# palash1992/GEM

Hardware: NVIDIA H100
Metric: nodes/sec embedded at d=128 (higher is better)
Workload: dtype f32

## Files before the change

### gem_b200/csrc/apply_tc.cu

```cuda
#include "tc_common.cuh"

namespace gemb {

struct ApplyTcParams {
    int64_t n;
    const float *Q;
    const float *M;
    float *Out;
    int b1, b2, ldm, ldo;
    uint32_t a_lbo;
    uint32_t a_tile;
    uint32_t b_tile;
    uint32_t raw_slot;
};

template <int TILE_M, int NPAD>
__global__ void __launch_bounds__(384, 1) apply_tc_kernel(ApplyTcParams p) {
    extern __shared__ __align__(128) char smem[];
    __shared__ __align__(8) uint64_t s_full[2], s_tile_full, s_tile_free;
    const int tid = threadIdx.x, lane = tid & 31, warp = tid >> 5;
    const int kchunks = p.b1 / 4;
    const int ksteps = p.b1 / 8;
    const uint32_t a_sbo = 128u;
    const uint32_t b_lbo = 128u;
    const uint32_t b_sbo = (uint32_t)kchunks * 128u;
    char *raw_base = smem;
    char *a_hi = smem + 2 * (size_t)p.raw_slot, *a_lo = a_hi + p.a_tile;
    char *b_hi = a_lo + p.a_tile, *b_lo = b_hi + p.b_tile;

    if (tid == 0) {
        for (int i = 0; i < 2; i++) tc::mbar_init(tc::smem_u32(&s_full[i]), 1);
        tc::mbar_init(tc::smem_u32(&s_tile_full), 4);
        tc::mbar_init(tc::smem_u32(&s_tile_free), 8);
        asm volatile("fence.mbarrier_init.release.cluster;" ::: "memory");
    }
    for (int idx = tid; idx < NPAD * kchunks; idx += blockDim.x) {
        const int nn = idx % NPAD, kc = idx / NPAD;
        float4 v = make_float4(0.f, 0.f, 0.f, 0.f);
        if (nn < p.b2) {
            const float *m = p.M + (size_t)(4 * kc) * p.ldm + nn;
            v = make_float4(__ldg(m), __ldg(m + p.ldm), __ldg(m + 2 * (size_t)p.ldm), __ldg(m + 3 * (size_t)p.ldm));
        }
        uint4 hi, lo;
        tc::split_tf32(v, hi, lo);
        const uint32_t off = (uint32_t)(nn >> 3) * b_sbo + (uint32_t)(nn & 7) * 16u + (uint32_t)kc * b_lbo;
        *(uint4 *)(b_hi + off) = hi;
        *(uint4 *)(b_lo + off) = lo;
    }
    tc::fence_proxy_async();
    __syncthreads();

    const int64_t tiles_total = (p.n + TILE_M - 1) / TILE_M;
    const int nt = (int)((tiles_total - blockIdx.x + gridDim.x - 1) / gridDim.x);
    auto tile_row0 = [&](int t) { return ((int64_t)blockIdx.x + (int64_t)t * gridDim.x) * TILE_M; };
    auto tile_rows = [&](int t) { const int64_t r0 = tile_row0(t); return (int)(p.n - r0 < TILE_M ? p.n - r0 : TILE_M); };

    if (warp >= 8) {
        auto issue = [&](int t) {
            const int slot = t & 1;
            const uint32_t bytes = (uint32_t)tile_rows(t) * (uint32_t)p.b1 * 4u;
            const uint32_t bar = tc::smem_u32(&s_full[slot]);
            tc::mbar_expect_tx(bar, bytes);
            tc::bulk_g2s(tc::smem_u32(raw_base + (size_t)slot * p.raw_slot), p.Q + tile_row0(t) * p.b1, bytes, bar);
        };
        if (tid == 256) {
            if (nt > 0) issue(0);
            if (nt > 1) issue(1);
        }
        const int ltid = tid - 256;
        for (int t = 0; t < nt; t++) {
            const int slot = t & 1;
            const char *raw = raw_base + (size_t)slot * p.raw_slot;
            tc::mbar_wait(tc::smem_u32(&s_full[slot]), (uint32_t)(t >> 1) & 1);
            if (t >= 1) tc::mbar_wait(tc::smem_u32(&s_tile_free), (uint32_t)(t - 1) & 1);
            const int vr = tile_rows(t);
            for (int idx = ltid; idx < TILE_M * kchunks; idx += 128) {
                const int m = idx / kchunks, kc = idx - m * kchunks;
                float4 v = make_float4(0.f, 0.f, 0.f, 0.f);
                if (m < vr) v = *(const float4 *)(raw + ((size_t)m * p.b1 + 4 * kc) * 4);
                uint4 hi, lo;
                tc::split_tf32(v, hi, lo);
                const uint32_t off = (uint32_t)(m >> 3) * a_sbo + (uint32_t)(m & 7) * 16u + (uint32_t)kc * p.a_lbo;
                *(uint4 *)(a_hi + off) = hi;
                *(uint4 *)(a_lo + off) = lo;
            }
            tc::fence_proxy_async();
            __syncwarp();
            if (lane == 0) tc::mbar_arrive(tc::smem_u32(&s_tile_full));
            tc::named_sync(1, 128);
            if (tid == 256 && t + 2 < nt) issue(t + 2);
        }
    } else {
        const int wg = warp >> 2;
        const bool active = wg * 64 < TILE_M;
        float acc[NPAD / 2];
        const uint32_t a_off = (uint32_t)wg * 8u * a_sbo;
        for (int t = 0; t < nt; t++) {
            tc::mbar_wait(tc::smem_u32(&s_tile_full), (uint32_t)t & 1);
            __syncwarp();
            uint64_t dah = tc::make_desc(tc::smem_u32(a_hi) + a_off, p.a_lbo, a_sbo), dal = tc::make_desc(tc::smem_u32(a_lo) + a_off, p.a_lbo, a_sbo);
            uint64_t dbh = tc::make_desc(tc::smem_u32(b_hi), b_lbo, b_sbo), dbl = tc::make_desc(tc::smem_u32(b_lo), b_lbo, b_sbo);
            const uint64_t a_step = (uint64_t)((2u * p.a_lbo) >> 4), b_step = (uint64_t)((2u * b_lbo) >> 4);
            if (active) {
                tc::wgmma_fence();
                for (int ks = 0; ks < ksteps; ks++) {
                    tc::wgmma_tf32<NPAD>(acc, dah, dbh, ks > 0 ? 1u : 0u);
                    tc::wgmma_tf32<NPAD>(acc, dah, dbl, 1u);
                    tc::wgmma_tf32<NPAD>(acc, dal, dbh, 1u);
                    dah += a_step; dal += a_step; dbh += b_step; dbl += b_step;
                }
                tc::wgmma_commit();
                tc::wgmma_wait_all();
            }
            __syncwarp();
            if (lane == 0) tc::mbar_arrive(tc::smem_u32(&s_tile_free));
            if (!active) continue;
            const int vr = tile_rows(t);
            const int r0 = wg * 64 + (warp & 3) * 16 + (lane >> 2);
            float *orow = p.Out + tile_row0(t) * p.ldo;
#pragma unroll
            for (int j = 0; j < NPAD / 8; j++) {
                const int col = j * 8 + (lane & 3) * 2;
                if (col < p.b2) {
                    if (r0 < vr) *(float2 *)(orow + (size_t)r0 * p.ldo + col) = make_float2(acc[4 * j], acc[4 * j + 1]);
                    if (r0 + 8 < vr) *(float2 *)(orow + (size_t)(r0 + 8) * p.ldo + col) = make_float2(acc[4 * j + 2], acc[4 * j + 3]);
                }
            }
        }
    }
}

template <int TILE_M, int NPAD>
static int apply_tc_launch_t(gemb_ctx *ctx, const ApplyTcParams &p, int grid, size_t smem_bytes) {
    static size_t attr_bytes = 0;
    if (attr_bytes < smem_bytes) {
        GEMB_CUDA(cudaFuncSetAttribute(apply_tc_kernel<TILE_M, NPAD>, cudaFuncAttributeMaxDynamicSharedMemorySize, (int)smem_bytes));
        attr_bytes = smem_bytes;
    }
    apply_tc_kernel<TILE_M, NPAD><<<grid, 384, smem_bytes, ctx->stream>>>(p);
    GEMB_CUDA(cudaGetLastError());
    count_launch();
    return GEMB_OK;
}

template <int TILE_M>
static int apply_tc_dispatch(gemb_ctx *ctx, const ApplyTcParams &p, int npad, int grid, size_t smem_bytes) {
    switch (npad) {
        case 32: return apply_tc_launch_t<TILE_M, 32>(ctx, p, grid, smem_bytes);
        case 64: return apply_tc_launch_t<TILE_M, 64>(ctx, p, grid, smem_bytes);
        case 80: return apply_tc_launch_t<TILE_M, 80>(ctx, p, grid, smem_bytes);
        case 96: return apply_tc_launch_t<TILE_M, 96>(ctx, p, grid, smem_bytes);
        default: return apply_tc_launch_t<TILE_M, 128>(ctx, p, grid, smem_bytes);
    }
}

static int pad_width(int b) {
    const int widths[5] = {32, 64, 80, 96, 128};
    for (int w : widths) if (w >= b) return w;
    return 128;
}

static size_t apply_smem_bytes(int tile_m, int b1, int npad) {
    const size_t raw_slot = (size_t)tile_m * b1 * 4, a_tile = (size_t)(b1 / 4) * (16 * tile_m + 16);
    const size_t b_tile = (size_t)(npad / 8) * (b1 / 4) * 128;
    return 2 * raw_slot + 2 * a_tile + 2 * b_tile + 256;
}

int apply_tc_launch(gemb_ctx *ctx, int64_t n, const float *Q, int b1, const float *M, int ldm, int b2, float *Out, int ldo) {
    if (b1 % 8 || b2 % 4 || b1 > 128 || ldo < b2 || ldo % 4 || ((uintptr_t)Out & 15) || n <= 0) return GEMB_ERR_UNSUPPORTED;
    const int cfg[5][2] = {{128, 128}, {64, 128}, {128, 64}, {64, 64}, {64, 32}};
    int tile_m = 0, nbw = 0;
    for (const auto &c : cfg) {
        const int w = std::min(c[1], b2);
        if (apply_smem_bytes(c[0], b1, pad_width(w)) <= 226 * 1024) { tile_m = c[0]; nbw = w; break; }
    }
    if (!tile_m) return GEMB_ERR_UNSUPPORTED;
    const int64_t tiles = (n + tile_m - 1) / tile_m;
    int grid = ctx->sm_count;
    if (grid > tiles) grid = (int)tiles;
    for (int n0 = 0; n0 < b2; n0 += nbw) {
        ApplyTcParams p;
        const int w = std::min(nbw, b2 - n0), npad = pad_width(w);
        p.n = n; p.Q = Q; p.M = M + n0; p.Out = Out + n0; p.b1 = b1; p.b2 = w; p.ldm = ldm; p.ldo = ldo;
        p.a_lbo = 16u * (uint32_t)tile_m + 16u;
        p.a_tile = (uint32_t)(b1 / 4) * p.a_lbo;
        p.b_tile = (uint32_t)(npad / 8) * (uint32_t)(b1 / 4) * 128u;
        p.raw_slot = (uint32_t)((size_t)tile_m * b1 * 4);
        const size_t smem_bytes = apply_smem_bytes(tile_m, b1, npad);
        if (tile_m == 128) GEMB_TRY(apply_tc_dispatch<128>(ctx, p, npad, grid, smem_bytes));
        else GEMB_TRY(apply_tc_dispatch<64>(ctx, p, npad, grid, smem_bytes));
    }
    return GEMB_OK;
}

}
```

### gem_b200/csrc/gram_tc.cu

```cuda
#include "tc_common.cuh"

namespace gemb {

struct GramTcParams {
    int64_t n;
    const float *P, *Q;
    int ldp, ldq;
    int m0, n0, mb, nb;
    double *part;
    int ldg;
    int64_t part_stride;
    int stage_rows;
    uint32_t tile_bytes_a, tile_bytes_b;
    uint32_t raw_bytes_p, raw_bytes_q;
};

__device__ __forceinline__ void transform_unit(const char *raw, int ld, int c0, int w, int valid_rows, int k4, int j32,
                                               int lane, char *tile_hi, char *tile_lo, uint32_t lbo, uint32_t sbo) {
    const int mn = j32 * 32 + lane;
    if (mn >= w) return;
    const int k0 = k4 * 4;
    const float *src = (const float *)raw + (size_t)k0 * ld + c0 + mn;
    float4 v;
    v.x = (k0 + 0 < valid_rows) ? src[0] : 0.f;
    v.y = (k0 + 1 < valid_rows) ? src[(size_t)ld] : 0.f;
    v.z = (k0 + 2 < valid_rows) ? src[2 * (size_t)ld] : 0.f;
    v.w = (k0 + 3 < valid_rows) ? src[3 * (size_t)ld] : 0.f;
    uint4 hi, lo;
    tc::split_tf32(v, hi, lo);
    const uint32_t off = (uint32_t)(mn >> 3) * sbo + (uint32_t)(mn & 7) * 16u + (uint32_t)k4 * lbo;
    *(uint4 *)(tile_hi + off) = hi;
    *(uint4 *)(tile_lo + off) = lo;
}

template <bool QRAW, bool BSEP, int NPAD>
__global__ void __launch_bounds__(384, 1) gram_tc_kernel(GramTcParams p) {
    extern __shared__ __align__(128) char smem[];
    __shared__ __align__(8) uint64_t s_full[3], s_tile_full[2], s_tile_free[2];
    const int tid = threadIdx.x, lane = tid & 31, warp = tid >> 5;
    const int kblocks = p.stage_rows / 8;
    const int kquads = p.stage_rows / 4;
    const uint32_t lbo = 128u;
    const uint32_t sbo = (uint32_t)kquads * 128u;
    const uint32_t raw_stage = p.raw_bytes_p + (QRAW ? p.raw_bytes_q : 0);
    const uint32_t stage_bytes = 2 * p.tile_bytes_a + (BSEP ? 2 * p.tile_bytes_b : 0);
    char *raw_base = smem;
    char *tile_base = smem + 3 * (size_t)raw_stage;

    if (tid == 0) {
        for (int i = 0; i < 2; i++) { tc::mbar_init(tc::smem_u32(&s_tile_full[i]), 4); tc::mbar_init(tc::smem_u32(&s_tile_free[i]), 8); }
        for (int i = 0; i < 3; i++) tc::mbar_init(tc::smem_u32(&s_full[i]), 1);
        asm volatile("fence.mbarrier_init.release.cluster;" ::: "memory");
    }
    __syncthreads();

    const int64_t stages_total = (p.n + p.stage_rows - 1) / p.stage_rows;
    const int64_t per_cta = (stages_total + gridDim.x - 1) / gridDim.x;
    const int64_t s_begin = (int64_t)blockIdx.x * per_cta;
    const int64_t s_end = s_begin + per_cta < stages_total ? s_begin + per_cta : stages_total;
    const int nst = (int)(s_end > s_begin ? s_end - s_begin : 0);

    if (warp >= 8) {
        const int lw = warp - 8;
        auto issue = [&](int it) {
            const int slot = it % 3;
            const int64_t row0 = (s_begin + it) * p.stage_rows;
            const int64_t vr = p.n - row0 < p.stage_rows ? p.n - row0 : p.stage_rows;
            const uint32_t bytes_p = (uint32_t)(vr * p.ldp * 4), bytes_q = QRAW ? (uint32_t)(vr * p.ldq * 4) : 0u;
            const uint32_t bar = tc::smem_u32(&s_full[slot]);
            char *dst = raw_base + (size_t)slot * raw_stage;
            tc::mbar_expect_tx(bar, bytes_p + bytes_q);
            tc::bulk_g2s(tc::smem_u32(dst), p.P + row0 * p.ldp, bytes_p, bar);
            if (QRAW) tc::bulk_g2s(tc::smem_u32(dst + p.raw_bytes_p), p.Q + row0 * p.ldq, bytes_q, bar);
        };
        if (tid == 256)
            for (int it = 0; it < 3 && it < nst; it++) issue(it);
        for (int it = 0; it < nst; it++) {
            const int st = it & 1, slot = it % 3;
            char *base = tile_base + (size_t)st * stage_bytes;
            const char *raw = raw_base + (size_t)slot * raw_stage;
            tc::mbar_wait(tc::smem_u32(&s_full[slot]), (uint32_t)(it / 3) & 1);
            if (it >= 2) tc::mbar_wait(tc::smem_u32(&s_tile_free[st]), (uint32_t)((it >> 1) - 1) & 1);
            const int64_t row0 = (s_begin + it) * p.stage_rows;
            const int vr = (int)(p.n - row0 < p.stage_rows ? p.n - row0 : p.stage_rows);
            const int units_a = kquads * ((p.mb + 31) / 32);
#pragma unroll 3
            for (int u = lw; u < units_a; u += 4)
                transform_unit(raw, p.ldp, p.m0, p.mb, vr, u % kquads, u / kquads, lane, base, base + p.tile_bytes_a, lbo, sbo);
            if (BSEP) {
                const int units_b = kquads * ((p.nb + 31) / 32);
                char *qb = base + 2 * p.tile_bytes_a;
                const char *rb = QRAW ? raw + p.raw_bytes_p : raw;
                const int ldb = QRAW ? p.ldq : p.ldp;
#pragma unroll 3
                for (int u = lw; u < units_b; u += 4)
                    transform_unit(rb, ldb, p.n0, p.nb, vr, u % kquads, u / kquads, lane, qb, qb + p.tile_bytes_b, lbo, sbo);
            }
            tc::fence_proxy_async();
            __syncwarp();
            if (lane == 0) tc::mbar_arrive(tc::smem_u32(&s_tile_full[st]));
            tc::named_sync(1, 128);
            if (tid == 256 && it + 3 < nst) issue(it + 3);
        }
    } else {
        const int wg = warp >> 2;
        const bool active = wg * 64 < p.mb;
        float acc[NPAD / 2], racc[NPAD / 2];
#pragma unroll
        for (int i = 0; i < NPAD / 2; i++) racc[i] = 0.f;
        for (int it = 0; it < nst; it++) {
            const int st = it & 1;
            tc::mbar_wait(tc::smem_u32(&s_tile_full[st]), (uint32_t)(it >> 1) & 1);
            if (active) {
                const uint32_t a_hi = tc::smem_u32(tile_base + (size_t)st * stage_bytes), a_lo = a_hi + p.tile_bytes_a;
                const uint32_t b_hi = BSEP ? a_hi + 2 * p.tile_bytes_a : a_hi;
                const uint32_t b_lo = BSEP ? b_hi + p.tile_bytes_b : a_lo;
                const uint32_t a_off = (uint32_t)wg * 8u * sbo;
                uint64_t dah = tc::make_desc(a_hi + a_off, lbo, sbo), dal = tc::make_desc(a_lo + a_off, lbo, sbo);
                uint64_t dbh = tc::make_desc(b_hi, lbo, sbo), dbl = tc::make_desc(b_lo, lbo, sbo);
                const uint64_t step = (uint64_t)((2u * lbo) >> 4);
                tc::wgmma_fence();
                for (int kb = 0; kb < kblocks; kb++) {
                    tc::wgmma_tf32<NPAD>(acc, dah, dbh, kb > 0 ? 1u : 0u);
                    tc::wgmma_tf32<NPAD>(acc, dah, dbl, 1u);
                    tc::wgmma_tf32<NPAD>(acc, dal, dbh, 1u);
                    dah += step; dal += step; dbh += step; dbl += step;
                }
                tc::wgmma_commit();
                tc::wgmma_wait_all();
            }
            __syncwarp();
            if (lane == 0) tc::mbar_arrive(tc::smem_u32(&s_tile_free[st]));
            if (active) {
#pragma unroll
                for (int i = 0; i < NPAD / 2; i++) racc[i] += acc[i];
            }
        }
        if (active) {
            const int r0 = wg * 64 + (warp & 3) * 16 + (lane >> 2);
            double *dst = p.part + (size_t)blockIdx.x * p.part_stride + (size_t)p.m0 * p.ldg + p.n0;
#pragma unroll
            for (int i = 0; i < NPAD / 2; i++) {
                const int row = r0 + ((i >> 1) & 1) * 8, col = (i >> 2) * 8 + (lane & 3) * 2 + (i & 1);
                if (row < p.mb && col < p.nb) dst[(size_t)row * p.ldg + col] = (double)racc[i];
            }
        }
    }
}

template <bool QRAW, bool BSEP, int NPAD>
static int gram_tc_launch_t(gemb_ctx *ctx, const GramTcParams &p, int grid, size_t smem_bytes) {
    static size_t attr_bytes = 0;
    if (attr_bytes < smem_bytes) {
        GEMB_CUDA(cudaFuncSetAttribute(gram_tc_kernel<QRAW, BSEP, NPAD>, cudaFuncAttributeMaxDynamicSharedMemorySize, (int)smem_bytes));
        attr_bytes = smem_bytes;
    }
    gram_tc_kernel<QRAW, BSEP, NPAD><<<grid, 384, smem_bytes, ctx->stream>>>(p);
    GEMB_CUDA(cudaGetLastError());
    count_launch();
    return GEMB_OK;
}

template <bool QRAW, bool BSEP>
static int gram_tc_dispatch(gemb_ctx *ctx, const GramTcParams &p, int grid, size_t smem_bytes) {
    if (p.nb <= 32) return gram_tc_launch_t<QRAW, BSEP, 32>(ctx, p, grid, smem_bytes);
    if (p.nb <= 64) return gram_tc_launch_t<QRAW, BSEP, 64>(ctx, p, grid, smem_bytes);
    if (p.nb <= 80) return gram_tc_launch_t<QRAW, BSEP, 80>(ctx, p, grid, smem_bytes);
    if (p.nb <= 96) return gram_tc_launch_t<QRAW, BSEP, 96>(ctx, p, grid, smem_bytes);
    return gram_tc_launch_t<QRAW, BSEP, 128>(ctx, p, grid, smem_bytes);
}

int gram_tc_launch(gemb_ctx *ctx, int64_t n, const float *P, int b1, const float *Q, int b2, double *G) {
    const bool cross = (P != Q);
    if (b1 % 4 || b2 % 4 || n <= 0) return GEMB_ERR_UNSUPPORTED;
    const int bm = (b1 + 127) / 128, bn = (b2 + 127) / 128;
    const size_t cols_raw = (size_t)b1 + (cross ? b2 : 0);
    size_t cols_tile = 0;
    for (int i = 0; i < bm; i++)
        for (int j = 0; j < bn; j++) {
            const int mb = std::min(128, b1 - 128 * i), nb = std::min(128, b2 - 128 * j);
            const bool bsep = cross || i != j;
            cols_tile = std::max(cols_tile, (size_t)(mb + 7) / 8 * 8 + (bsep ? (size_t)(nb + 7) / 8 * 8 : 0));
        }
    const size_t bytes_per_row = 3 * 4 * cols_raw + 2 * 2 * 4 * cols_tile;
    int rows = (int)((176 * 1024) / bytes_per_row) / 8 * 8;
    if (rows > 64) rows = 64;
    if (rows < 8) return GEMB_ERR_UNSUPPORTED;
    const size_t sbo = (size_t)(rows / 4) * 128;
    const size_t raw_stage = (size_t)rows * cols_raw * 4;
    const size_t smem_bytes = 3 * raw_stage + 2 * cols_tile / 8 * 2 * sbo + 16 * sbo + 1024;
    if (smem_bytes > 226 * 1024) return GEMB_ERR_UNSUPPORTED;
    const int64_t stages_total = (n + rows - 1) / rows;
    int grid = ctx->sm_count;
    if (grid > stages_total) grid = (int)stages_total;
    double *part = nullptr;
    GEMB_TRY(red_scratch(ctx, (size_t)grid * b1 * b2, &part));
    GramTcParams p;
    p.n = n; p.P = P; p.Q = Q; p.ldp = b1; p.ldq = b2;
    p.part = part; p.ldg = b2; p.part_stride = (int64_t)b1 * b2;
    p.stage_rows = rows;
    p.raw_bytes_p = (uint32_t)(rows * b1 * 4);
    p.raw_bytes_q = (uint32_t)(rows * b2 * 4);
    for (int i = 0; i < bm; i++)
        for (int j = 0; j < bn; j++) {
            p.m0 = 128 * i; p.mb = std::min(128, b1 - p.m0);
            p.n0 = 128 * j; p.nb = std::min(128, b2 - p.n0);
            p.tile_bytes_a = (uint32_t)((p.mb + 7) / 8) * (uint32_t)(rows / 4) * 128u;
            p.tile_bytes_b = (uint32_t)((p.nb + 7) / 8) * (uint32_t)(rows / 4) * 128u;
            if (cross) GEMB_TRY((gram_tc_dispatch<true, true>(ctx, p, grid, smem_bytes)));
            else if (i != j) GEMB_TRY((gram_tc_dispatch<false, true>(ctx, p, grid, smem_bytes)));
            else GEMB_TRY((gram_tc_dispatch<false, false>(ctx, p, grid, smem_bytes)));
        }
    return sum_partials_launch(ctx, grid, (int64_t)b1 * b2, part, G);
}

}
```

### gem_b200/csrc/hope.cu

```cuda
#include "common.cuh"
#include <chrono>
#include "nccl_api.h"
#include <math.h>
#include <string.h>
#include <algorithm>
#include <numeric>

namespace gemb {

struct HopeWork {
    gemb_graph *g;
    gemb_ctx *c;
    int b;
    int64_t rows;
    int64_t shard;
    float *buf[5] = {nullptr, nullptr, nullptr, nullptr, nullptr};
    float *full = nullptr;
    double *G = nullptr, *G2 = nullptr, *w = nullptr, *Z = nullptr, *Zs = nullptr, *scal = nullptr;
    float *Minv = nullptr, *M1 = nullptr, *M2 = nullptr;
    int *rank_dev = nullptr;
    int64_t spmm_wide = 0, spmm_all = 0;
    bool halo = false;
    int64_t pushes = 0;
    double push_bytes_per_row = 0.0;
    bool wire_half = false;
    bool wire_full_now = false;
    bool blk_half[5] = {false, false, false, false, false};
    bool push_half() const { return wire_half && !wire_full_now; }
    int buf_index(const float *p) const { for (int i = 0; i < 5; i++) if (buf[i] == p) return i; return -1; }
    ~HopeWork() {
        if (!halo) for (auto p : buf) dfree(p);
        dfree(full); dfree(G); dfree(G2); dfree(w); dfree(Z); dfree(Zs); dfree(scal);
        dfree(Minv); dfree(M1); dfree(M2); dfree(rank_dev);
    }
};

struct HopeResult {
    int iters = 0, converged = 0, katz_terms = 0, algorithm = 0;
    double change = 0.0;
    float resid_max = -1.f, resid_est = -1.f;
    float *Xd = nullptr;
    float *Xalloc = nullptr;
    float *sig_dev = nullptr;
    double sigma_max = 0.0;
};

static int comm_allgather(HopeWork &W, const float *shard_src, int width) {
    NcclApi *api = nccl_api();
    if (!api) return GEMB_ERR_NCCL;
    GEMB_TRY(W.c->t_comm.begin(W.c->stream));
    ncclResult_t r = api->AllGather(shard_src, W.full, (size_t)W.shard * width, ncclFloat,
                                    (ncclComm_t)W.c->comm, W.c->stream);
    if (r != ncclSuccess) { set_error("ncclAllGather: %s", api->GetErrorString(r)); return GEMB_ERR_NCCL; }
    GEMB_TRY(W.c->t_comm.end(W.c->stream));
    return GEMB_OK;
}

static int comm_allreduce_f64(HopeWork &W, double *buf, size_t count) {
    if (W.c->nranks == 1) return GEMB_OK;
    NcclApi *api = nccl_api();
    if (!api) return GEMB_ERR_NCCL;
    GEMB_TRY(W.c->t_comm.begin(W.c->stream));
    ncclResult_t r = api->AllReduce(buf, buf, count, ncclDouble, ncclSum, (ncclComm_t)W.c->comm, W.c->stream);
    if (r != ncclSuccess) { set_error("ncclAllReduce: %s", api->GetErrorString(r)); return GEMB_ERR_NCCL; }
    GEMB_TRY(W.c->t_comm.end(W.c->stream));
    return GEMB_OK;
}

static int publish(HopeWork &W, const float *buf, int width) {
    if (!W.halo) return GEMB_OK;
    const int bi = W.buf_index(buf);
    GEMB_ARG(bi >= 0, "publish: not a work block");
    const bool half = W.push_half();
    GEMB_TRY(W.c->t_comm.begin(W.c->stream));
    GEMB_TRY(halo_push_launch(W.g, bi, width, half));
    GEMB_TRY(halo_barrier(W.g));
    GEMB_TRY(W.c->t_comm.end(W.c->stream));
    W.blk_half[bi] = half;
    W.pushes++;
    W.push_bytes_per_row += (half ? 2.0 : 4.0) * width;
    return GEMB_OK;
}

static int dist_spmm3(HopeWork &W, bool transpose, int width, float alpha, const float *Xshard, float gamma,
                      bool use_self, float delta, const float *X0, float *Y, bool timed, bool push_out = false) {
    if (W.halo) {
        gemb_csr_dev A = W.g->A;
        A.indices = W.g->halo.indices_ext;
        HaloPushArgs P;
        const int bo = W.buf_index(Y), bin = W.buf_index(Xshard);
        GEMB_ARG(bin >= 0, "spmm input is not a work block");
        const bool half_out = W.push_half();
        if (push_out) { GEMB_ARG(bo >= 0, "spmm output is not a work block"); halo_push_args(W.g, bo, &P, half_out); }
        if (timed) GEMB_TRY(W.c->t_spmm.begin(W.c->stream));
        GEMB_TRY(spmm3_launch(W.c, A, W.rows, width, alpha, Xshard, gamma, use_self ? Xshard : nullptr, delta, X0, Y,
                              push_out ? &P : nullptr, W.blk_half[bin] ? W.g->n_shard : 0));
        if (timed) { GEMB_TRY(W.c->t_spmm.end(W.c->stream)); W.spmm_wide++; }
        W.spmm_all++;
        if (push_out) {
            GEMB_TRY(W.c->t_comm.begin(W.c->stream));
            GEMB_TRY(halo_barrier(W.g));
            GEMB_TRY(W.c->t_comm.end(W.c->stream));
            W.blk_half[bo] = half_out;
            W.pushes++;
            W.push_bytes_per_row += (half_out ? 2.0 : 4.0) * width;
        }
        return GEMB_OK;
    }
    const float *Xfull = Xshard;
    if (W.c->nranks > 1) {
        GEMB_TRY(comm_allgather(W, Xshard, width));
        Xfull = W.full;
    }
    if (timed) GEMB_TRY(W.c->t_spmm.begin(W.c->stream));
    GEMB_TRY(spmm3_launch(W.c, transpose ? W.g->AT : W.g->A, W.rows, width, alpha, Xfull, gamma,
                          use_self ? Xshard : nullptr, delta, X0, Y));
    if (timed) { GEMB_TRY(W.c->t_spmm.end(W.c->stream)); W.spmm_wide++; }
    W.spmm_all++;
    return GEMB_OK;
}

static int dist_spmm(HopeWork &W, bool transpose, int width, float alpha, const float *Xshard,
                     const float *X0, float *Y, bool timed) {
    return dist_spmm3(W, transpose, width, alpha, Xshard, 0.f, false, 1.f, X0, Y, timed);
}

static int katz(HopeWork &W, bool transpose, float beta, int J, const float *in, float *out,
                float *t1, float *t2) {
    const float *cur = in;
    for (int m = 1; m <= J; m++) {
        if (m < J) {
            float *dst = (m & 1) ? t1 : t2;
            GEMB_TRY(dist_spmm3(W, transpose, W.b, beta, cur, 0.f, false, 1.f, in, dst, true, W.halo));
            cur = dst;
        } else {
            GEMB_TRY(dist_spmm(W, transpose, W.b, beta, cur, nullptr, out, true));
        }
    }
    return GEMB_OK;
}

static int gram_full(HopeWork &W, const float *P, const float *Q, double *G) {
    GEMB_TRY(W.c->t_dense.begin(W.c->stream));
    GEMB_TRY(gram_launch(W.c, W.rows, P, W.b, Q, W.b, G));
    GEMB_TRY(W.c->t_dense.end(W.c->stream));
    GEMB_TRY(comm_allreduce_f64(W, G, (size_t)W.b * W.b));
    return GEMB_OK;
}

static int cholqr_pass(HopeWork &W, double *G, const float *src, float *dst) {
    GEMB_TRY(W.c->t_dense.begin(W.c->stream));
    GEMB_TRY(chol_inverse_launch(W.c, W.b, G, W.Minv, W.rank_dev));
    GEMB_TRY(apply_launch(W.c, W.rows, src, W.b, W.Minv, W.b, W.b, dst, W.b));
    GEMB_TRY(W.c->t_dense.end(W.c->stream));
    return GEMB_OK;
}

static int cholqr2(HopeWork &W, const float *src, float *tmp, float *dst) {
    GEMB_TRY(gram_full(W, src, src, W.G));
    GEMB_TRY(cholqr_pass(W, W.G, src, tmp));
    GEMB_TRY(gram_full(W, tmp, tmp, W.G));
    GEMB_TRY(cholqr_pass(W, W.G, tmp, dst));
    return GEMB_OK;
}

__global__ void ritz_maps_kernel(int b, int k, const double *__restrict__ w, const double *__restrict__ Z,
                                 float *__restrict__ M1, float *__restrict__ M2, double p1, double p2,
                                 double rel_floor = 1e-28) {
    const int idx = blockIdx.x * blockDim.x + threadIdx.x;
    if (idx >= b * k) return;
    const int i = idx / k, j = idx - i * k;
    const double wmax = w[b - 1];
    const double th = w[b - k + j];
    const double z = Z[(size_t)i * b + (b - k + j)];
    double a = 0.0, c = 0.0;
    if (th > rel_floor * wmax && th > 0.0) { a = z * pow(th, p1); c = z * pow(th, p2); }
    M1[idx] = (float)a;
    M2[idx] = (float)c;
}

__global__ void sqrt_top_kernel(int b, int k, const double *__restrict__ w, float *__restrict__ sigma) {
    const int j = blockIdx.x * blockDim.x + threadIdx.x;
    if (j < k) { const double th = w[b - k + j]; sigma[j] = (float)(th > 0.0 ? sqrt(th) : 0.0); }
}

__global__ void coldiff_sumsq_kernel(int64_t n, int b, const float *__restrict__ A, const float *__restrict__ B,
                                     double *__restrict__ out) {
    const int j = threadIdx.x % b;
    const int rpb = blockDim.x / b;
    double acc = 0.0;
    for (int64_t r = (int64_t)blockIdx.x * rpb + threadIdx.x / b; r < n; r += (int64_t)gridDim.x * rpb) {
        const double d = (double)A[r * b + j] - (double)B[r * b + j];
        acc += d * d;
    }
    atomicAdd(out + j, acc);
}

__global__ void symmetrize_kernel(int b, double *__restrict__ T) {
    const int idx = blockIdx.x * blockDim.x + threadIdx.x;
    if (idx >= b * b) return;
    const int i = idx / b, j = idx - i * b;
    if (i < j) {
        const double v = 0.5 * (T[(size_t)i * b + j] + T[(size_t)j * b + i]);
        T[(size_t)i * b + j] = v;
        T[(size_t)j * b + i] = v;
    }
}

__global__ void axpby_kernel(int64_t count, float a, const float4 *__restrict__ P, float c,
                             const float4 *__restrict__ Q, float4 *__restrict__ Y) {
    for (int64_t i = (int64_t)blockIdx.x * blockDim.x + threadIdx.x; i < count; i += (int64_t)gridDim.x * blockDim.x) {
        const float4 p = P[i], q = Q[i];
        Y[i] = make_float4(a * p.x + c * q.x, a * p.y + c * q.y, a * p.z + c * q.z, a * p.w + c * q.w);
    }
}

__global__ void __launch_bounds__(256)
axpby_push_kernel(int64_t n_rows, int G, int rows_per_cta, float a, const float4 *__restrict__ P, float c,
                  const float4 *__restrict__ Q, float4 *__restrict__ Y, HaloPushArgs H) {
    const int lr = threadIdx.x / G, cc = threadIdx.x - lr * G;
    if (lr >= rows_per_cta) return;
    const int64_t row = (int64_t)blockIdx.x * rows_per_cta + lr;
    if (row >= n_rows) return;
    const float4 p = P[row * G + cc], q = Q[row * G + cc];
    const float4 v = make_float4(a * p.x + c * q.x, a * p.y + c * q.y, a * p.z + c * q.z, a * p.w + c * q.w);
    Y[row * G + cc] = v;
    halo_push_row(H, row, G, cc, v);
}

static int axpby_launch(HopeWork &W, float a, const float *P, float c, const float *Q, float *Y) {
    const int64_t count = W.rows * (int64_t)W.b / 4;
    if (W.halo) {
        const int G = W.b / 4, rpc = 256 / G, bo = W.buf_index(Y);
        GEMB_ARG(bo >= 0 && G <= 256, "axpby output is not a work block");
        HaloPushArgs H;
        const bool half = W.push_half();
        halo_push_args(W.g, bo, &H, half);
        W.blk_half[bo] = half;
        W.push_bytes_per_row += (half ? 2.0 : 4.0) * W.b;
        if (W.rows > 0) {
            axpby_push_kernel<<<(unsigned)((W.rows + rpc - 1) / rpc), 256, 0, W.c->stream>>>(
                W.rows, G, rpc, a, (const float4 *)P, c, (const float4 *)Q, (float4 *)Y, H);
            GEMB_CUDA(cudaGetLastError());
            count_launch();
        }
        GEMB_TRY(W.c->t_comm.begin(W.c->stream));
        GEMB_TRY(halo_barrier(W.g));
        GEMB_TRY(W.c->t_comm.end(W.c->stream));
        W.pushes++;
        return GEMB_OK;
    }
    if (count == 0) return GEMB_OK;
    int grid = W.c->sm_count * 8;
    if ((int64_t)grid * 256 > count) grid = (int)((count + 255) / 256);
    axpby_kernel<<<grid, 256, 0, W.c->stream>>>(count, a, (const float4 *)P, c, (const float4 *)Q, (float4 *)Y);
    GEMB_CUDA(cudaGetLastError());
    count_launch();
    return GEMB_OK;
}

__global__ void csr_rowsum_kernel(int64_t n, const int32_t *__restrict__ indptr, const float *__restrict__ vals,
                                  double *__restrict__ out) {
    double mx = 0.0, neg = 0.0;
    for (int64_t r = (int64_t)blockIdx.x * blockDim.x + threadIdx.x; r < n; r += (int64_t)gridDim.x * blockDim.x) {
        const int s = indptr[r], e = indptr[r + 1];
        double acc = 0.0;
        if (vals) {
            for (int i = s; i < e; i++) { const double v = vals[i]; acc += fabs(v); if (-v > neg) neg = -v; }
        } else acc = (double)(e - s);
        if (acc > mx) mx = acc;
    }
    for (int o = 16; o > 0; o >>= 1) {
        mx = fmax(mx, __shfl_xor_sync(0xffffffffu, mx, o));
        neg = fmax(neg, __shfl_xor_sync(0xffffffffu, neg, o));
    }
    if ((threadIdx.x & 31) == 0) {
        atomicMax((unsigned long long *)out, (unsigned long long)__double_as_longlong(mx));
        atomicMax((unsigned long long *)(out + 1), (unsigned long long)__double_as_longlong(neg));
    }
}

static int comm_allreduce_max_f64(HopeWork &W, double *buf, size_t count) {
    if (W.c->nranks == 1) return GEMB_OK;
    NcclApi *api = nccl_api();
    if (!api) return GEMB_ERR_NCCL;
    ncclResult_t r = api->AllReduce(buf, buf, count, ncclDouble, ncclMax, (ncclComm_t)W.c->comm, W.c->stream);
    if (r != ncclSuccess) { set_error("ncclAllReduce(max): %s", api->GetErrorString(r)); return GEMB_ERR_NCCL; }
    return GEMB_OK;
}

static int rowsum_bound(HopeWork &W, double *norm_inf, bool *nonneg) {
    gemb_ctx *c = W.c;
    GEMB_CUDA(cudaMemsetAsync(W.scal, 0, 2 * sizeof(double), c->stream));
    if (W.rows > 0) {
        csr_rowsum_kernel<<<c->sm_count * 8, 256, 0, c->stream>>>(W.rows, W.g->A.indptr, W.g->A.data, W.scal);
        GEMB_CUDA(cudaGetLastError());
        count_launch();
    }
    GEMB_TRY(comm_allreduce_max_f64(W, W.scal, 2));
    double h[2];
    GEMB_CUDA(cudaMemcpyAsync(h, W.scal, sizeof h, cudaMemcpyDeviceToHost, c->stream));
    GEMB_CUDA(cudaStreamSynchronize(c->stream));
    *norm_inf = h[0];
    *nonneg = (h[1] == 0.0);
    return GEMB_OK;
}

static int estimate_norm2(HopeWork &W, uint64_t seed, float *x, float *y, float *z, double *out) {
    gemb_ctx *c = W.c;
    gemb_graph *g = W.g;
    const int pw = 4;
    struct FullWire { HopeWork &w; bool old; FullWire(HopeWork &w_) : w(w_), old(w_.wire_full_now) { w.wire_full_now = true; } ~FullWire() { w.wire_full_now = old; } } fw(W);
    GEMB_TRY(randn_launch(c, W.rows, pw, seed ^ 0x5bd1e995u, (uint64_t)g->row0, x));
    double est = 0.0, prev = -1.0;
    for (int it = 0; it < 16; it++) {
        double h[2];
        GEMB_TRY(sumsq_launch(c, W.rows * pw, x, W.scal));
        GEMB_TRY(publish(W, x, pw));
        GEMB_TRY(dist_spmm3(W, false, pw, 1.f, x, 0.f, false, 1.f, nullptr, y, false, true));
        GEMB_TRY(dist_spmm(W, true, pw, 1.f, y, nullptr, z, false));
        GEMB_TRY(sumsq_launch(c, W.rows * pw, z, W.scal + 1));
        GEMB_TRY(comm_allreduce_f64(W, W.scal, 2));
        GEMB_CUDA(cudaMemcpyAsync(h, W.scal, sizeof h, cudaMemcpyDeviceToHost, c->stream));
        GEMB_CUDA(cudaStreamSynchronize(c->stream));
        if (!(h[0] > 0.0) || !(h[1] > 0.0)) { est = 0.0; break; }
        est = sqrt(sqrt(h[1] / h[0]));
        GEMB_TRY(scale_launch(c, W.rows * pw, (float)(1.0 / sqrt(h[1])), z));
        std::swap(x, z);
        if (prev > 0 && fabs(est - prev) <= 1e-3 * est && it >= 3) break;
        prev = est;
    }
    *out = est;
    return GEMB_OK;
}

static int probe_katz_terms(HopeWork &W, float beta, double katz_tol, uint64_t seed, float *x, float *y, int *J_out,
                            double *rho_est) {
    gemb_ctx *c = W.c;
    const int pw = 4, Jmax = 2048;
    int Jbest = 1;
    *rho_est = 0.0;
    for (int tr = 0; tr < 2; tr++) {
        GEMB_TRY(randn_launch(c, W.rows, pw, seed ^ (0x7f4a7c15u + tr), (uint64_t)W.g->row0, x));
        double peak = 0.0, prev = 0.0;
        int j = 0;
        bool done = false;
        for (j = 1; j <= Jmax; j++) {
            double h = 0.0;
            GEMB_TRY(dist_spmm(W, tr == 1, pw, beta, x, nullptr, y, false));
            GEMB_TRY(sumsq_launch(c, W.rows * pw, y, W.scal));
            GEMB_TRY(comm_allreduce_f64(W, W.scal, 1));
            GEMB_CUDA(cudaMemcpyAsync(&h, W.scal, sizeof h, cudaMemcpyDeviceToHost, c->stream));
            GEMB_CUDA(cudaStreamSynchronize(c->stream));
            const double nt = sqrt(h);
            if (prev > 0.0) *rho_est = std::max(*rho_est * (j > 8 ? 0.0 : 1.0), nt / prev / (double)beta);
            if (!(nt < 1e30)) break;
            peak = std::max(peak, nt);
            if (nt <= katz_tol * peak) { done = true; break; }
            prev = nt;
            std::swap(x, y);
        }
        if (!done) return GEMB_ERR_DIVERGE;
        Jbest = std::max(Jbest, j);
    }
    *J_out = std::min(4096, Jbest + Jbest / 8 + 2);
    return GEMB_OK;
}

struct Opts {
    int oversample = 16, max_iters = 30, min_iters = 2, katz_terms = 0, compute_residual = 0, verbose = 0;
    int algorithm = 0, cheb_degree = 8, stop_rule = 0, lanczos_basis = 0;
    int spectral_mode = 0;
    float tol = 1e-6f, katz_tol = 1e-7f, range_log2 = 8.f;
    uint64_t seed = 1234;
};

static int katz_terms_for(double beta, double nrm, double katz_tol) {
    const double x1 = beta * nrm * 1.02;
    if (x1 <= 1e-30) return 1;
    int J = (int)ceil(log(katz_tol) / log(x1));
    return std::max(1, std::min(J, 4096));
}

static int residual_check(HopeWork &W, float beta, int J, const float *P, const float *Qs, float *scr0, float *scr1,
                          float *scr2, const std::vector<int> &cols, double smax, float *out) {
    gemb_ctx *c = W.c;
    const int b = W.b;
    GEMB_TRY(katz(W, true, beta, J, P, scr0, scr1, scr2));
    GEMB_CUDA(cudaMemsetAsync(W.scal, 0, sizeof(double) * b, c->stream));
    const int threads = (256 / b) * b > 0 ? (256 / b) * b : b;
    coldiff_sumsq_kernel<<<c->sm_count * 4, threads, 0, c->stream>>>(W.rows, b, scr0, Qs, W.scal);
    GEMB_CUDA(cudaGetLastError());
    count_launch();
    GEMB_TRY(comm_allreduce_f64(W, W.scal, b));
    std::vector<double> rs(b);
    GEMB_CUDA(cudaMemcpyAsync(rs.data(), W.scal, sizeof(double) * b, cudaMemcpyDeviceToHost, c->stream));
    GEMB_CUDA(cudaStreamSynchronize(c->stream));
    double rm = 0.0;
    for (int j : cols) rm = std::max(rm, sqrt(rs[j]) / std::max(smax, 1e-300));
    *out = (float)rm;
    return GEMB_OK;
}

static int hope_general(HopeWork &W, const Opts &o, int d, float beta, int J, HopeResult &R) {
    gemb_ctx *c = W.c;
    const int b = W.b, k = d / 2;
    float *V = W.buf[0], *U = W.buf[1], *Wk = W.buf[2], *T1 = W.buf[3], *T2 = W.buf[4];
    R.algorithm = 1;
    R.katz_terms = J;
    GEMB_TRY(randn_launch(c, W.rows, b, o.seed, (uint64_t)W.g->row0, T1));
    GEMB_TRY(cholqr2(W, T1, T2, V));

    std::vector<double> theta(b), theta_prev(b, 0.0);
    for (int it = 1; it <= o.max_iters; it++) {
        R.iters = it;
        GEMB_TRY(katz(W, false, beta, J, V, U, T1, T2));
        GEMB_TRY(gram_full(W, U, U, W.G));
        GEMB_CUDA(cudaMemcpyAsync(W.G2, W.G, sizeof(double) * b * b, cudaMemcpyDeviceToDevice, c->stream));
        GEMB_TRY(c->t_dense.begin(c->stream));
        GEMB_TRY(eigh_launch(c, b, W.G2, W.w, W.Z, W.Zs, std::min(1e-5, std::max(1e-13, 1e-2 * (double)o.tol))));
        GEMB_TRY(c->t_dense.end(c->stream));
        GEMB_CUDA(cudaMemcpyAsync(theta.data(), W.w, sizeof(double) * b, cudaMemcpyDeviceToHost, c->stream));
        GEMB_CUDA(cudaStreamSynchronize(c->stream));
        const double tmax = std::max(theta[b - 1], 1e-300);
        double change = 0.0;
        for (int j = b - k; j < b; j++) {
            const double sj = sqrt(std::max(theta[j], 0.0)), sp = sqrt(std::max(theta_prev[j], 0.0));
            change = std::max(change, fabs(sj - sp) / std::max(sj, 1e-3 * sqrt(tmax)));
        }
        R.change = change;
        theta_prev = theta;
        if (o.verbose)
            fprintf(stderr, "[gemb_hope/general] it %d  sigma_max %.6g sigma_k %.6g  ritz change %.3g\n", it,
                    sqrt(tmax), sqrt(std::max(theta[b - k], 0.0)), change);
        if (it >= o.min_iters && change <= (double)o.tol) { R.converged = 1; break; }
        if (it == o.max_iters) break;
        GEMB_TRY(c->t_dense.begin(c->stream));
        ritz_maps_kernel<<<(b * b + 255) / 256, 256, 0, c->stream>>>(b, b, W.w, W.Z, W.M1, W.M2, -0.5, 0.5, 1e-10);
        GEMB_CUDA(cudaGetLastError());
        count_launch();
        GEMB_TRY(apply_launch(c, W.rows, U, b, W.M1, b, b, T1, b));
        GEMB_TRY(c->t_dense.end(c->stream));
        GEMB_TRY(katz(W, true, beta, J, T1, Wk, U, T2));
        GEMB_TRY(cholqr2(W, Wk, T1, V));
    }
    R.sigma_max = sqrt(std::max(theta[b - 1], 0.0));

    R.Xd = T1;
    if ((size_t)d > (size_t)b) {
        GEMB_CUDA(dmalloc(&R.Xalloc, sizeof(float) * (size_t)std::max<int64_t>(W.rows, 1) * d));
        R.Xd = R.Xalloc;
    }
    GEMB_TRY(c->t_dense.begin(c->stream));
    ritz_maps_kernel<<<(b * k + 255) / 256, 256, 0, c->stream>>>(b, k, W.w, W.Z, W.M1, W.M2, -0.25, 0.25);
    GEMB_CUDA(cudaGetLastError());
    count_launch();
    GEMB_TRY(apply_launch(c, W.rows, U, b, W.M1, k, k, R.Xd, d));
    GEMB_TRY(apply_launch(c, W.rows, V, b, W.M2, k, k, R.Xd + k, d));
    R.sig_dev = (float *)W.G2;
    sqrt_top_kernel<<<(k + 127) / 128, 128, 0, c->stream>>>(b, k, W.w, R.sig_dev);
    GEMB_CUDA(cudaGetLastError());
    count_launch();
    GEMB_TRY(c->t_dense.end(c->stream));

    if (o.compute_residual) {
        ritz_maps_kernel<<<(b * b + 255) / 256, 256, 0, c->stream>>>(b, b, W.w, W.Z, W.M1, W.M2, -0.5, 0.5);
        GEMB_CUDA(cudaGetLastError());
        count_launch();
        float *Pm = Wk, *Qs = nullptr, *Qalloc = nullptr, *STP = nullptr;
        const size_t blk = sizeof(float) * (size_t)W.shard * b;
        if (R.Xalloc) Qs = T1;
        else { GEMB_CUDA(dmalloc(&Qalloc, blk ? blk : 4)); GEMB_CUDA(cudaMemsetAsync(Qalloc, 0, blk, c->stream)); Qs = Qalloc; }
        GEMB_CUDA(dmalloc(&STP, blk ? blk : 4));
        GEMB_CUDA(cudaMemsetAsync(STP, 0, blk, c->stream));
        int s = apply_launch(c, W.rows, U, b, W.M1, b, b, Pm, b);
        if (s == GEMB_OK) s = apply_launch(c, W.rows, V, b, W.M2, b, b, Qs, b);
        std::vector<int> cols;
        for (int j = b - k; j < b; j++) cols.push_back(j);
        if (s == GEMB_OK) s = residual_check(W, beta, J, Pm, Qs, STP, U, T2, cols, R.sigma_max, &R.resid_max);
        dfree(STP);
        dfree(Qalloc);
        if (s != GEMB_OK) return s;
    }
    return GEMB_OK;
}

static int orth_rotated(HopeWork &W, const float *F, float *tmp, float *dst) {
    gemb_ctx *c = W.c;
    const int b = W.b;
    GEMB_TRY(gram_full(W, F, F, W.G));
    GEMB_TRY(c->t_dense.begin(c->stream));
    GEMB_TRY(small_gemm_launch(c, b, W.G, 0, W.Z, W.Zs, nullptr));
    GEMB_TRY(small_gemm_launch(c, b, W.Z, 1, W.Zs, W.G, nullptr));
    GEMB_TRY(chol_inverse_launch(c, b, W.G, W.Minv, W.rank_dev, W.G2));
    GEMB_TRY(small_gemm_launch(c, b, W.Z, 0, W.G2, nullptr, W.M1));
    GEMB_TRY(apply_launch(c, W.rows, F, b, W.M1, b, b, tmp, b));
    GEMB_TRY(c->t_dense.end(c->stream));
    GEMB_TRY(gram_full(W, tmp, tmp, W.G));
    GEMB_TRY(cholqr_pass(W, W.G, tmp, dst));
    return GEMB_OK;
}

__global__ void refill_cols_kernel(int64_t count, int b, const double *__restrict__ G, const float *__restrict__ Rn,
                                   float *__restrict__ V) {
    for (int64_t i = (int64_t)blockIdx.x * blockDim.x + threadIdx.x; i < count; i += (int64_t)gridDim.x * blockDim.x) {
        const int j = (int)(i % b);
        if (G[(size_t)j * b + j] < 0.5) V[i] = Rn[i];
    }
}

static int refill_dropped(HopeWork &W, float *V, float *s1, float *s2, uint64_t seed) {
    gemb_ctx *c = W.c;
    const int b = W.b;
    int rank = b;
    GEMB_CUDA(cudaMemcpyAsync(&rank, W.rank_dev, sizeof(int), cudaMemcpyDeviceToHost, c->stream));
    GEMB_CUDA(cudaStreamSynchronize(c->stream));
    if (rank >= b) return GEMB_OK;
    GEMB_TRY(randn_launch(c, W.rows, b, seed, (uint64_t)W.g->row0, s1));
    GEMB_TRY(gram_full(W, V, V, W.G));
    const int64_t count = W.rows * (int64_t)b;
    if (count > 0) {
        const int grid = (int)std::min<int64_t>((count + 255) / 256, (int64_t)c->sm_count * 8);
        refill_cols_kernel<<<grid, 256, 0, c->stream>>>(count, b, W.G, s1, V);
        GEMB_CUDA(cudaGetLastError());
        count_launch();
    }
    GEMB_TRY(gram_full(W, V, V, W.G));
    GEMB_TRY(cholqr_pass(W, W.G, V, s2));
    GEMB_TRY(gram_full(W, s2, s2, W.G));
    GEMB_TRY(cholqr_pass(W, W.G, s2, V));
    return GEMB_OK;
}

static inline double katz_f(double beta, double l) { return beta * l / (1.0 - beta * l); }
constexpr int GEMB_SWITCH_TO_LANCZOS = 1000;

static int hope_symmetric(HopeWork &W, const Opts &o, int d, float beta, double nrm, double hard_bound, HopeResult &R) {
    gemb_ctx *c = W.c;
    const int mode = o.spectral_mode;
    const int b = W.b, k = mode ? d : d / 2;
    R.algorithm = 2;
    R.katz_terms = 0;
    float *V = W.buf[0], *AV = W.buf[1];
    float *pool[3] = {W.buf[2], W.buf[3], W.buf[4]};
    const bool ritz_bound = nrm < 0.0;
    double bound = ritz_bound ? hard_bound * 1.02 + 1e-30 : nrm * 1.02 + 1e-30;

    bool careful = getenv("GEMB_WARMUP_CAREFUL") != nullptr;
    if (!careful) {
        W.wire_full_now = true;
        GEMB_TRY(randn_launch(c, W.rows, b, o.seed, (uint64_t)W.g->row0, pool[0]));
        GEMB_TRY(publish(W, pool[0], b));
        GEMB_TRY(dist_spmm3(W, false, b, 1.f, pool[0], 0.f, false, 1.f, nullptr, pool[1], true, W.halo));
        GEMB_TRY(dist_spmm3(W, false, b, 1.f, pool[1], 0.f, false, 1.f, nullptr, pool[2], true, W.halo));
        GEMB_TRY(dist_spmm(W, false, b, 1.f, pool[2], nullptr, AV, true));
        W.wire_full_now = false;
        GEMB_TRY(gram_full(W, AV, AV, W.G));
        GEMB_TRY(cholqr_pass(W, W.G, AV, pool[0]));
        int rank1 = b;
        GEMB_CUDA(cudaMemcpyAsync(&rank1, W.rank_dev, sizeof(int), cudaMemcpyDeviceToHost, c->stream));
        GEMB_CUDA(cudaStreamSynchronize(c->stream));
        if (rank1 < b) careful = true;
        else {
            GEMB_TRY(gram_full(W, pool[0], pool[0], W.G));
            GEMB_TRY(cholqr_pass(W, W.G, pool[0], V));
            GEMB_TRY(publish(W, V, b));
        }
    }
    if (careful) {
        GEMB_TRY(randn_launch(c, W.rows, b, o.seed, (uint64_t)W.g->row0, pool[0]));
        GEMB_TRY(cholqr2(W, pool[0], pool[1], V));
        GEMB_TRY(publish(W, V, b));
        for (int s = 0; s < 3; s++) {
            GEMB_TRY(dist_spmm(W, false, b, 1.f, V, nullptr, AV, true));
            GEMB_TRY(cholqr2(W, AV, pool[0], V));
            GEMB_TRY(publish(W, V, b));
        }
    }

    std::vector<double> lam(b), gval(b), th_sorted(b), th_prev(b, 0.0);
    std::vector<double> Wh(o.stop_rule == 1 ? (size_t)b * b : 0), Zr(o.stop_rule == 1 ? (size_t)b * b : 0);
    std::vector<int> order(b);
    struct Plan { bool valid = false; int deg = 0; double e = 0, c0 = 0, sigma1 = 0; } plan;

    auto run_filter = [&](const Plan &pl, float **out) -> int {
        double sigma = pl.sigma1;
        const double e = pl.e, c0 = pl.c0, tau2 = 2.0 / pl.sigma1;
        float *prev = V, *cur = pool[0];
        float *free_a = pool[1], *free_b = pool[2];
        GEMB_TRY(axpby_launch(W, (float)(sigma / e), AV, (float)(-sigma * c0 / e), V, cur));
        for (int i = 2; i <= pl.deg; i++) {
            const double sn = 1.0 / (tau2 - sigma);
            float *nxt = free_a;
            GEMB_TRY(dist_spmm3(W, false, b, (float)(2.0 * sn / e), cur, (float)(-2.0 * sn * c0 / e), true,
                                (float)(-sigma * sn), prev, nxt, true, i < pl.deg));
            sigma = sn;
            float *old_prev = prev;
            prev = cur;
            cur = nxt;
            if (old_prev == V) { free_a = free_b; free_b = nullptr; }
            else { free_a = old_prev; }
        }
        *out = cur;
        return GEMB_OK;
    };

    for (int it = 1; it <= o.max_iters; it++) {
        R.iters = it;
        GEMB_TRY(dist_spmm(W, false, b, 1.f, V, nullptr, AV, true));
        GEMB_TRY(gram_full(W, V, AV, W.G2));
        symmetrize_kernel<<<(b * b + 255) / 256, 256, 0, c->stream>>>(b, W.G2);
        GEMB_CUDA(cudaGetLastError());
        count_launch();
        GEMB_TRY(c->t_dense.begin(c->stream));
        GEMB_TRY(eigh_launch(c, b, W.G2, W.w, W.Z, W.Zs, std::min(1e-5, std::max(1e-13, 1e-2 * (double)o.tol))));
        GEMB_TRY(c->t_dense.end(c->stream));
        GEMB_CUDA(cudaMemcpyAsync(lam.data(), W.w, sizeof(double) * b, cudaMemcpyDeviceToHost, c->stream));
        GEMB_CUDA(cudaStreamSynchronize(c->stream));
        float *filtered = nullptr;
        if (ritz_bound) {
            double amax = 0.0;
            for (int i = 0; i < b; i++) amax = std::max(amax, fabs(lam[i]));
            bound = std::min(hard_bound * 1.02, 1.05 * amax) + 1e-30;
        }
        for (int i = 0; i < b; i++) {
            const double l = std::max(-bound, std::min(bound, lam[i]));
            gval[i] = mode ? (l + bound) : fabs(katz_f(beta, l));
        }
        std::iota(order.begin(), order.end(), 0);
        std::sort(order.begin(), order.end(), [&](int a, int c2) { return gval[a] > gval[c2]; });
        for (int i = 0; i < b; i++) th_sorted[i] = gval[order[i]] * gval[order[i]];
        const double tmax = std::max(th_sorted[0], 1e-300);
        double change = 0.0;
        for (int j = 0; j < k; j++) {
            const double sj = sqrt(th_sorted[j]), sp = sqrt(th_prev[j]);
            change = std::max(change, fabs(sj - sp) / std::max(sj, 1e-3 * sqrt(tmax)));
        }
        R.change = change;
        th_prev = th_sorted;
        if (it == 1 && !mode && o.algorithm == 0 && W.g->n >= 2048 && gval[order[k - 1]] < 0.33 * gval[order[0]] &&
            gval[order[std::min(b - 1, 3)]] < 0.7 * gval[order[0]])
            return GEMB_SWITCH_TO_LANCZOS;
        double stop_measure = change;
        if (o.stop_rule == 1) {
            GEMB_TRY(gram_full(W, AV, AV, W.G));
            GEMB_CUDA(cudaMemcpyAsync(Wh.data(), W.G, sizeof(double) * b * b, cudaMemcpyDeviceToHost, c->stream));
            GEMB_CUDA(cudaMemcpyAsync(Zr.data(), W.Z, sizeof(double) * b * b, cudaMemcpyDeviceToHost, c->stream));
            GEMB_CUDA(cudaStreamSynchronize(c->stream));
            double worst = 0.0;
            for (int j = 0; j < k; j++) {
                const int col = order[j];
                double q = 0.0;
                for (int r = 0; r < b; r++) {
                    double t = 0.0;
                    for (int s2 = 0; s2 < b; s2++) t += Wh[(size_t)r * b + s2] * Zr[(size_t)s2 * b + col];
                    q += Zr[(size_t)r * b + col] * t;
                }
                const double l = std::max(-bound, std::min(bound, lam[col]));
                const double r2 = std::max(q - lam[col] * lam[col], 0.0);
                const double fp = mode ? 1.0 : (double)beta / ((1.0 - beta * l) * (1.0 - beta * l));
                worst = std::max(worst, fp * sqrt(r2) / std::max(gval[order[0]], 1e-300));
            }
            stop_measure = worst;
            R.resid_est = (float)worst;
        }
        if (o.verbose)
            fprintf(stderr, "[gemb_hope/symmetric] it %d  sigma_max %.6g sigma_k %.6g  ritz change %.3g%s%.3g\n", it,
                    gval[order[0]], gval[order[k - 1]], change, o.stop_rule == 1 ? "  residual " : " ", o.stop_rule == 1 ? stop_measure : 0.0);
        if (it >= o.min_iters && stop_measure <= (double)o.tol) { R.converged = 1; break; }
        if (it == o.max_iters) break;

        const double tau = gval[order[b - 1]];
        double hi = mode ? std::max(-bound, std::min(bound, lam[order[b - 1]])) : tau / ((double)beta * (1.0 + tau));
        double lo = mode ? -bound : (tau < 1.0 ? -tau / ((double)beta * (1.0 - tau)) : -bound);
        lo = std::max(lo, -bound);
        hi = std::min(hi, bound);
        if (hi - lo < 2e-3 * bound) { const double mid = 0.5 * (hi + lo); lo = mid - 1e-3 * bound; hi = mid + 1e-3 * bound; }
        Plan np;
        np.valid = true;
        np.e = 0.5 * (hi - lo);
        np.c0 = 0.5 * (hi + lo);
        const double aL = (mode || lam[order[0]] >= np.c0) ? bound : -bound;
        np.sigma1 = np.e / (aL - np.c0);
        const double xL = fabs(aL - np.c0) / np.e;
        const double growth = xL + sqrt(std::max(xL * xL - 1.0, 0.0));
        np.deg = o.cheb_degree;
        const double range_log2 = getenv("GEMB_CHEB_RANGE_LOG2") ? atof(getenv("GEMB_CHEB_RANGE_LOG2")) : (double)o.range_log2;
        if (growth > 1.0 + 1e-9) np.deg = std::min(np.deg, (int)floor(log(2.0 * exp2(range_log2)) / log(growth)));

        if (!filtered) {
            if (np.deg < 2) {
                GEMB_TRY(orth_rotated(W, AV, pool[0], V));
                GEMB_TRY(refill_dropped(W, V, pool[0], pool[1], o.seed + 7919ull * (uint64_t)it));
                GEMB_TRY(publish(W, V, b));
                plan = np;
                continue;
            }
            GEMB_TRY(run_filter(np, &filtered));
        }
        plan = np;
        float *tmp = nullptr;
        for (float *cand : {pool[0], pool[1], pool[2], AV})
            if (cand != filtered) { tmp = cand; break; }
        GEMB_TRY(orth_rotated(W, filtered, tmp, V));
        GEMB_TRY(refill_dropped(W, V, tmp, filtered, o.seed + 7919ull * (uint64_t)it));
        GEMB_TRY(publish(W, V, b));
    }

    if (mode) {
        std::vector<double> Zh((size_t)b * b);
        GEMB_CUDA(cudaMemcpyAsync(Zh.data(), W.Z, sizeof(double) * b * b, cudaMemcpyDeviceToHost, c->stream));
        GEMB_CUDA(cudaStreamSynchronize(c->stream));
        std::vector<float> M1((size_t)b * k), ev(k);
        for (int j = 0; j < k; j++) {
            const int col = order[j];
            ev[j] = (float)std::max(-bound, std::min(bound, lam[col]));
            for (int i = 0; i < b; i++) M1[(size_t)i * k + j] = (float)Zh[(size_t)i * b + col];
        }
        R.sigma_max = gval[order[0]];
        GEMB_CUDA(cudaMemcpyAsync(W.M1, M1.data(), sizeof(float) * b * k, cudaMemcpyHostToDevice, c->stream));
        R.sig_dev = (float *)W.G2;
        GEMB_CUDA(cudaMemcpyAsync(R.sig_dev, ev.data(), sizeof(float) * k, cudaMemcpyHostToDevice, c->stream));
        GEMB_CUDA(cudaStreamSynchronize(c->stream));
        R.Xd = pool[0];
        GEMB_TRY(c->t_dense.begin(c->stream));
        GEMB_TRY(apply_launch(c, W.rows, V, b, W.M1, k, k, R.Xd, k));
        GEMB_TRY(c->t_dense.end(c->stream));
        return GEMB_OK;
    }
    std::vector<int> sel(order.begin(), order.begin() + k);
    std::reverse(sel.begin(), sel.end());
    std::vector<double> Zh((size_t)b * b);
    GEMB_CUDA(cudaMemcpyAsync(Zh.data(), W.Z, sizeof(double) * b * b, cudaMemcpyDeviceToHost, c->stream));
    GEMB_CUDA(cudaStreamSynchronize(c->stream));
    std::vector<float> M1((size_t)b * k), M2((size_t)b * k), sig(k);
    for (int j = 0; j < k; j++) {
        const int col = sel[j];
        const double l = std::max(-bound, std::min(bound, lam[col]));
        const double f = katz_f(beta, l), sg = fabs(f), rt = sqrt(sg);
        sig[j] = (float)sg;
        for (int i = 0; i < b; i++) {
            const double z = Zh[(size_t)i * b + col];
            M2[(size_t)i * k + j] = (float)(z * rt);
            M1[(size_t)i * k + j] = (float)((f < 0 ? -z : z) * rt);
        }
    }
    R.sigma_max = gval[order[0]];
    GEMB_CUDA(cudaMemcpyAsync(W.M1, M1.data(), sizeof(float) * b * k, cudaMemcpyHostToDevice, c->stream));
    GEMB_CUDA(cudaMemcpyAsync(W.M2, M2.data(), sizeof(float) * b * k, cudaMemcpyHostToDevice, c->stream));
    R.sig_dev = (float *)W.G2;
    GEMB_CUDA(cudaMemcpyAsync(R.sig_dev, sig.data(), sizeof(float) * k, cudaMemcpyHostToDevice, c->stream));
    GEMB_CUDA(cudaStreamSynchronize(c->stream));
    R.Xd = pool[0];
    if ((size_t)d > (size_t)b) {
        GEMB_CUDA(dmalloc(&R.Xalloc, sizeof(float) * (size_t)std::max<int64_t>(W.rows, 1) * d));
        R.Xd = R.Xalloc;
    }
    GEMB_TRY(c->t_dense.begin(c->stream));
    GEMB_TRY(apply_launch(c, W.rows, V, b, W.M1, k, k, R.Xd, d));
    GEMB_TRY(apply_launch(c, W.rows, V, b, W.M2, k, k, R.Xd + k, d));
    GEMB_TRY(c->t_dense.end(c->stream));

    if (o.compute_residual) {
        const int J = katz_terms_for(beta, ritz_bound ? bound / 1.02 : nrm, o.katz_tol);
        std::vector<float> MP((size_t)b * b, 0.f), MQ((size_t)b * b, 0.f);
        for (int col = 0; col < b; col++) {
            const double l = std::max(-bound, std::min(bound, lam[col]));
            const double f = katz_f(beta, l);
            for (int i = 0; i < b; i++) {
                const double z = Zh[(size_t)i * b + col];
                MP[(size_t)i * b + col] = (float)(f < 0 ? -z : z);
                MQ[(size_t)i * b + col] = (float)(z * fabs(f));
            }
        }
        float *dMP = nullptr, *dMQ = nullptr, *Palloc = nullptr, *Q = nullptr, *STP = nullptr;
        const size_t blk = sizeof(float) * (size_t)W.shard * b;
        GEMB_CUDA(dmalloc(&dMP, sizeof(float) * b * b));
        GEMB_CUDA(dmalloc(&dMQ, sizeof(float) * b * b));
        float *P = AV;
        if (!W.halo) { GEMB_CUDA(dmalloc(&Palloc, blk ? blk : 4)); GEMB_CUDA(cudaMemsetAsync(Palloc, 0, blk, c->stream)); P = Palloc; }
        GEMB_CUDA(dmalloc(&Q, blk ? blk : 4));
        GEMB_CUDA(dmalloc(&STP, blk ? blk : 4));
        GEMB_CUDA(cudaMemsetAsync(Q, 0, blk, c->stream));
        GEMB_CUDA(cudaMemsetAsync(STP, 0, blk, c->stream));
        GEMB_CUDA(cudaMemcpyAsync(dMP, MP.data(), sizeof(float) * b * b, cudaMemcpyHostToDevice, c->stream));
        GEMB_CUDA(cudaMemcpyAsync(dMQ, MQ.data(), sizeof(float) * b * b, cudaMemcpyHostToDevice, c->stream));
        W.wire_full_now = true;
        int s = apply_launch(c, W.rows, V, b, dMP, b, b, P, b);
        if (s == GEMB_OK) s = apply_launch(c, W.rows, V, b, dMQ, b, b, Q, b);
        if (s == GEMB_OK) s = publish(W, P, b);
        if (s == GEMB_OK) s = residual_check(W, beta, J, P, Q, STP, W.halo ? pool[1] : AV, W.halo ? pool[2] : pool[1], sel, R.sigma_max, &R.resid_max);
        cudaStreamSynchronize(c->stream);
        dfree(dMP); dfree(dMQ); dfree(Palloc); dfree(Q); dfree(STP);
        if (s != GEMB_OK) return s;
    }
    return GEMB_OK;
}

__global__ void put_cols_kernel(int64_t n, int w, const float *__restrict__ src, float *__restrict__ dst, int ldd, int col0) {
    for (int64_t i = (int64_t)blockIdx.x * blockDim.x + threadIdx.x; i < n * w; i += (int64_t)gridDim.x * blockDim.x) {
        const int64_t r = i / w;
        const int cc = (int)(i - r * w);
        dst[r * ldd + col0 + cc] = src[i];
    }
}
__global__ void reverse_put_kernel(int64_t n, int w, const float *__restrict__ src, int lds, float *__restrict__ dst, int ldd, int col_last) {
    for (int64_t i = (int64_t)blockIdx.x * blockDim.x + threadIdx.x; i < n * w; i += (int64_t)gridDim.x * blockDim.x) {
        const int64_t r = i / w;
        const int q = (int)(i - r * w);
        dst[r * ldd + col_last - q] = src[r * lds + q];
    }
}
__global__ void f64_to_f32_kernel(int count, const double *__restrict__ a, float *__restrict__ o) {
    const int i = blockIdx.x * blockDim.x + threadIdx.x;
    if (i < count) o[i] = (float)a[i];
}
__global__ void axpy_kernel(int64_t count, float a, const float *__restrict__ X, float *__restrict__ Y, int accumulate) {
    for (int64_t i = (int64_t)blockIdx.x * blockDim.x + threadIdx.x; i < count; i += (int64_t)gridDim.x * blockDim.x)
        Y[i] = accumulate ? fmaf(a, X[i], Y[i]) : a * X[i];
}

static int hope_lanczos(HopeWork &W, const Opts &o, int d, float beta, double hard_bound, HopeResult &R) {
    gemb_ctx *c = W.c;
    const int k = d / 2, p = 16, cw = 64;
    const int64_t rows = W.rows, shard = W.shard;
    R.algorithm = 3;
    R.katz_terms = 0;
    const int k_keep = (k + p + p - 1) / p * p;
    int m_max = o.lanczos_basis > 0 ? o.lanczos_basis : std::max(2 * k_keep, 160);
    m_max = (m_max + p - 1) / p * p;
    GEMB_ARG(m_max >= k_keep + 2 * p && m_max <= 1024, "algorithm3_basis");
    const int nchunk = (m_max + cw - 1) / cw;
    const int mt = m_max + p;
    const size_t chunk_bytes = sizeof(float) * (size_t)shard * cw;
    std::vector<float *> Q(nchunk, nullptr), Qn((k_keep + cw - 1) / cw, nullptr);
    struct Free { std::vector<float *> *a, *b; float *t[3]; double *g[3]; float *m32;
                  ~Free() { for (auto x : *a) dfree(x); for (auto x : *b) dfree(x); for (auto x : t) dfree(x); for (auto x : g) dfree(x); dfree(m32); } }
        guard{&Q, &Qn, {nullptr, nullptr, nullptr}, {nullptr, nullptr, nullptr}, nullptr};
    for (auto &q : Q) { GEMB_CUDA(dmalloc(&q, chunk_bytes ? chunk_bytes : 4)); GEMB_CUDA(cudaMemsetAsync(q, 0, chunk_bytes, c->stream)); }
    for (auto &q : Qn) { GEMB_CUDA(dmalloc(&q, chunk_bytes ? chunk_bytes : 4)); }
    float *Vcur = W.buf[0], *Wb = W.buf[1], *Tb = W.buf[2], *Tmp64 = nullptr;
    GEMB_CUDA(dmalloc(&guard.t[0], chunk_bytes ? chunk_bytes : 4));
    Tmp64 = guard.t[0];
    double *Gd = nullptr, *Td = nullptr, *Yd = nullptr;
    GEMB_CUDA(dmalloc(&guard.g[0], sizeof(double) * (size_t)cw * cw)); Gd = guard.g[0];
    GEMB_CUDA(dmalloc(&guard.g[1], sizeof(double) * (size_t)mt * mt)); Td = guard.g[1];
    GEMB_CUDA(dmalloc(&guard.g[2], sizeof(double) * (size_t)mt * mt)); Yd = guard.g[2];
    GEMB_CUDA(dmalloc(&guard.m32, sizeof(float) * (size_t)cw * cw));
    float *M32 = guard.m32;
    double *wd = nullptr, *Zs = nullptr;
    GEMB_CUDA(dmalloc(&wd, sizeof(double) * mt));
    GEMB_CUDA(dmalloc(&Zs, sizeof(double) * (size_t)mt * mt));
    struct Free2 { double *a, *b; ~Free2() { dfree(a); dfree(b); } } guard2{wd, Zs};

    const int grid_el = c->sm_count * 8;
    auto gram_ar = [&](const float *P, int b1, const float *Qp, int b2, double *G) -> int {
        GEMB_TRY(c->t_dense.begin(c->stream));
        GEMB_TRY(gram_launch(c, rows, P, b1, Qp, b2, G));
        GEMB_TRY(c->t_dense.end(c->stream));
        return comm_allreduce_f64(W, G, (size_t)b1 * b2);
    };
    std::vector<double> Rh((size_t)p * p), R1((size_t)p * p), R2((size_t)p * p), Ginv((size_t)p * p);
    auto cholqr_p = [&](float *src, float *scratch, double *Rout) -> int {
        for (int pass = 0; pass < 2; pass++) {
            GEMB_TRY(gram_ar(src, p, src, p, W.G));
            GEMB_TRY(c->t_dense.begin(c->stream));
            GEMB_TRY(chol_inverse_launch(c, p, W.G, W.Minv, W.rank_dev, W.G2));
            GEMB_TRY(apply_launch(c, rows, src, p, W.Minv, p, p, scratch, p));
            GEMB_TRY(c->t_dense.end(c->stream));
            GEMB_CUDA(cudaMemcpyAsync(src, scratch, sizeof(float) * (size_t)rows * p, cudaMemcpyDeviceToDevice, c->stream));
            GEMB_CUDA(cudaMemcpyAsync(Ginv.data(), W.G2, sizeof(double) * p * p, cudaMemcpyDeviceToHost, c->stream));
            GEMB_CUDA(cudaStreamSynchronize(c->stream));
            std::vector<double> &Rt = pass == 0 ? R1 : R2;
            std::fill(Rt.begin(), Rt.end(), 0.0);
            for (int j = 0; j < p; j++) {
                if (Ginv[(size_t)j * p + j] == 0.0) continue;
                Rt[(size_t)j * p + j] = 1.0 / Ginv[(size_t)j * p + j];
                for (int i = j - 1; i >= 0; i--) {
                    if (Ginv[(size_t)i * p + i] == 0.0) continue;
                    double sacc = 0.0;
                    for (int l = i + 1; l <= j; l++) sacc += Ginv[(size_t)i * p + l] * Rt[(size_t)l * p + j];
                    Rt[(size_t)i * p + j] = -sacc / Ginv[(size_t)i * p + i];
                }
            }
        }
        for (int i = 0; i < p; i++)
            for (int j = 0; j < p; j++) {
                double a = 0.0;
                for (int l = 0; l < p; l++) a += R2[(size_t)i * p + l] * R1[(size_t)l * p + j];
                Rout[(size_t)i * p + j] = a;
            }
        return GEMB_OK;
    };

    std::vector<double> T((size_t)mt * mt, 0.0), Hcol((size_t)m_max * p), Hc((size_t)cw * p), theta(m_max), Y((size_t)m_max * m_max);
    std::vector<double> fabsv(m_max);
    std::vector<int> order(m_max);
    GEMB_TRY(randn_launch(c, rows, p, o.seed, (uint64_t)W.g->row0, Vcur));
    GEMB_TRY(cholqr_p(Vcur, Tb, Rh.data()));
    int m = 0, restarts = 0, steps = 0;
    double bound = hard_bound * 1.02 + 1e-30;
    const int max_steps = std::max(o.max_iters, 1) * (m_max / p);
    bool done = false;
    while (!done) {
        put_cols_kernel<<<grid_el, 256, 0, c->stream>>>(rows, p, Vcur, Q[m / cw], cw, m % cw);
        GEMB_CUDA(cudaGetLastError());
        count_launch();
        const int j0 = m;
        m += p;
        steps++;
        GEMB_TRY(publish(W, Vcur, p));
        GEMB_TRY(dist_spmm3(W, false, p, 1.f, Vcur, 0.f, false, 1.f, nullptr, Wb, true, false));
        std::fill(Hcol.begin(), Hcol.end(), 0.0);
        const int nc_live = (m + cw - 1) / cw;
        for (int pass = 0; pass < 2; pass++) {
            for (int cc = 0; cc < nc_live; cc++) {
                GEMB_TRY(gram_ar(Q[cc], cw, Wb, p, Gd));
                GEMB_TRY(c->t_dense.begin(c->stream));
                f64_to_f32_kernel<<<(cw * p + 255) / 256, 256, 0, c->stream>>>(cw * p, Gd, M32);
                GEMB_CUDA(cudaGetLastError());
                GEMB_TRY(apply_launch(c, rows, Q[cc], cw, M32, p, p, Tb, p));
                axpy_kernel<<<grid_el, 256, 0, c->stream>>>(rows * (int64_t)p, -1.f, Tb, Wb, 1);
                GEMB_CUDA(cudaGetLastError());
                count_launch(2);
                GEMB_TRY(c->t_dense.end(c->stream));
                GEMB_CUDA(cudaMemcpyAsync(Hc.data(), Gd, sizeof(double) * cw * p, cudaMemcpyDeviceToHost, c->stream));
                GEMB_CUDA(cudaStreamSynchronize(c->stream));
                for (int r = 0; r < cw && cc * cw + r < m; r++)
                    for (int q = 0; q < p; q++) Hcol[(size_t)(cc * cw + r) * p + q] += Hc[(size_t)r * p + q];
            }
        }
        for (int r = 0; r < m; r++)
            for (int q = 0; q < p; q++) {
                const double v = Hcol[(size_t)r * p + q];
                T[(size_t)r * mt + j0 + q] = v;
                T[(size_t)(j0 + q) * mt + r] = v;
            }
        for (int a2 = 0; a2 < p; a2++)
            for (int b2 = a2 + 1; b2 < p; b2++) {
                const double v = 0.5 * (T[(size_t)(j0 + a2) * mt + j0 + b2] + T[(size_t)(j0 + b2) * mt + j0 + a2]);
                T[(size_t)(j0 + a2) * mt + j0 + b2] = v;
                T[(size_t)(j0 + b2) * mt + j0 + a2] = v;
            }
        GEMB_TRY(cholqr_p(Wb, Tb, Rh.data()));
        GEMB_CUDA(cudaMemcpyAsync(Vcur, Wb, sizeof(float) * (size_t)rows * p, cudaMemcpyDeviceToDevice, c->stream));
        const bool full = m + p > m_max;
        if (!full && steps < max_steps) continue;

        std::vector<double> Tm((size_t)m * m);
        for (int r = 0; r < m; r++) for (int q = 0; q < m; q++) Tm[(size_t)r * m + q] = T[(size_t)r * mt + q];
        GEMB_CUDA(cudaMemcpyAsync(Td, Tm.data(), sizeof(double) * m * m, cudaMemcpyHostToDevice, c->stream));
        GEMB_TRY(c->t_dense.begin(c->stream));
        GEMB_TRY(eigh_launch(c, m, Td, wd, Yd, Zs, 1e-9));
        GEMB_TRY(c->t_dense.end(c->stream));
        GEMB_CUDA(cudaMemcpyAsync(theta.data(), wd, sizeof(double) * m, cudaMemcpyDeviceToHost, c->stream));
        GEMB_CUDA(cudaMemcpyAsync(Y.data(), Yd, sizeof(double) * m * m, cudaMemcpyDeviceToHost, c->stream));
        GEMB_CUDA(cudaStreamSynchronize(c->stream));
        double amax = 0.0;
        for (int i = 0; i < m; i++) amax = std::max(amax, fabs(theta[i]));
        bound = std::min(hard_bound * 1.02, 1.02 * amax) + 1e-30;
        for (int i = 0; i < m; i++) fabsv[i] = fabs(katz_f(beta, std::max(-bound, std::min(bound, theta[i]))));
        std::iota(order.begin(), order.begin() + m, 0);
        std::sort(order.begin(), order.begin() + m, [&](int a2, int b2) { return fabsv[a2] > fabsv[b2]; });
        const double smax = std::max(fabsv[order[0]], 1e-300);
        double worst = 0.0;
        for (int jj = 0; jj < std::min(k, m); jj++) {
            const int col = order[jj];
            double r2 = 0.0;
            for (int a2 = 0; a2 < p; a2++) {
                double t = 0.0;
                for (int b2 = 0; b2 < p; b2++) t += Rh[(size_t)a2 * p + b2] * Y[(size_t)(m - p + b2) * m + col];
                r2 += t * t;
            }
            const double l = std::max(-bound, std::min(bound, theta[col]));
            const double fp = (double)beta / ((1.0 - beta * l) * (1.0 - beta * l));
            worst = std::max(worst, fp * sqrt(r2) / smax);
        }
        R.change = worst;
        R.resid_est = (float)worst;
        restarts++;
        R.iters = restarts;
        if (o.verbose)
            fprintf(stderr, "[gemb_hope/lanczos] restart %d  basis %d  steps %d  sigma_max %.6g sigma_k %.6g  residual %.3g\n", restarts, m,
                    steps, smax, fabsv[order[std::min(k, m) - 1]], worst);
        const bool conv = m >= k && worst <= (double)o.tol;
        if (conv) R.converged = 1;
        done = conv || steps >= max_steps;
        const int nk = done ? k : std::min(k_keep, m);
        const int ncn = (nk + cw - 1) / cw;
        for (int oc = 0; oc < ncn; oc++) {
            const int ow = std::min(cw, nk - oc * cw);
            for (int cc = 0; cc < nc_live; cc++) {
                std::vector<float> Mh((size_t)cw * cw, 0.f);
                for (int r = 0; r < cw && cc * cw + r < m; r++)
                    for (int q = 0; q < ow; q++) Mh[(size_t)r * cw + q] = (float)Y[(size_t)(cc * cw + r) * m + order[oc * cw + q]];
                GEMB_CUDA(cudaMemcpyAsync(M32, Mh.data(), sizeof(float) * cw * cw, cudaMemcpyHostToDevice, c->stream));
                GEMB_CUDA(cudaStreamSynchronize(c->stream));
                GEMB_TRY(c->t_dense.begin(c->stream));
                GEMB_TRY(apply_launch(c, rows, Q[cc], cw, M32, cw, cw, cc == 0 ? Qn[oc] : Tmp64, cw));
                if (cc > 0) {
                    axpy_kernel<<<grid_el, 256, 0, c->stream>>>(rows * (int64_t)cw, 1.f, Tmp64, Qn[oc], 1);
                    GEMB_CUDA(cudaGetLastError());
                    count_launch();
                }
                GEMB_TRY(c->t_dense.end(c->stream));
            }
        }
        if (done) {
            std::vector<float> sig(k);
            R.sigma_max = smax;
            R.Xd = nullptr;
            GEMB_CUDA(dmalloc(&R.Xalloc, sizeof(float) * (size_t)std::max<int64_t>(rows, 1) * d));
            R.Xd = R.Xalloc;
            GEMB_ARG(k <= cw * (int)Qn.size(), "k");
            std::vector<float> Ms((size_t)cw * cw), Mt((size_t)cw * cw);
            for (int oc = 0; oc < ncn; oc++) {
                const int ow = std::min(cw, k - oc * cw);
                std::fill(Ms.begin(), Ms.end(), 0.f); std::fill(Mt.begin(), Mt.end(), 0.f);
                for (int q = 0; q < ow; q++) {
                    const int jj = oc * cw + q, col = order[jj];
                    const double l = std::max(-bound, std::min(bound, theta[col]));
                    const double f = katz_f(beta, l), sg = fabs(f), rt = sqrt(sg);
                    sig[k - 1 - jj] = (float)sg;
                    Ms[(size_t)q * cw + q] = (float)(f < 0 ? -rt : rt);
                    Mt[(size_t)q * cw + q] = (float)rt;
                }
                for (int half = 0; half < 2; half++) {
                    GEMB_CUDA(cudaMemcpyAsync(M32, (half == 0 ? Ms : Mt).data(), sizeof(float) * cw * cw, cudaMemcpyHostToDevice, c->stream));
                    GEMB_CUDA(cudaStreamSynchronize(c->stream));
                    GEMB_TRY(apply_launch(c, rows, Qn[oc], cw, M32, cw, cw, Tmp64, cw));
                    reverse_put_kernel<<<grid_el, 256, 0, c->stream>>>(rows, ow, Tmp64, cw, R.Xd, d, half * k + k - 1 - oc * cw);
                    GEMB_CUDA(cudaGetLastError());
                    count_launch();
                }
            }
            R.sig_dev = (float *)W.G2;
            GEMB_CUDA(cudaMemcpyAsync(R.sig_dev, sig.data(), sizeof(float) * k, cudaMemcpyHostToDevice, c->stream));
            GEMB_CUDA(cudaStreamSynchronize(c->stream));
            break;
        }
        for (int oc = 0; oc < nchunk; oc++) {
            if (oc < ncn) GEMB_CUDA(cudaMemcpyAsync(Q[oc], Qn[oc], chunk_bytes, cudaMemcpyDeviceToDevice, c->stream));
            else GEMB_CUDA(cudaMemsetAsync(Q[oc], 0, chunk_bytes, c->stream));
        }
        std::fill(T.begin(), T.end(), 0.0);
        for (int q = 0; q < nk; q++) T[(size_t)q * mt + q] = theta[order[q]];
        m = nk;
    }
    return GEMB_OK;
}

__global__ void split_halves_kernel(int64_t n, int d, const float *__restrict__ X, float *__restrict__ L, float *__restrict__ Rr) {
    const int k = d / 2;
    for (int64_t i = (int64_t)blockIdx.x * blockDim.x + threadIdx.x; i < n * d; i += (int64_t)gridDim.x * blockDim.x) {
        const int64_t r = i / d;
        const int cc = (int)(i - r * d);
        if (cc < k) L[r * k + cc] = X[i]; else Rr[r * k + (cc - k)] = X[i];
    }
}
__global__ void probe_block_kernel(int64_t n, int w, int64_t p0, int probe, uint64_t seed, float *__restrict__ Z) {
    for (int64_t i = (int64_t)blockIdx.x * blockDim.x + threadIdx.x; i < n * w; i += (int64_t)gridDim.x * blockDim.x) {
        const int64_t r = i / w;
        const int cc = (int)(i - r * w);
        float v;
        if (probe) {
            uint64_t h = seed ^ ((uint64_t)r * 0x9E3779B97F4A7C15ull) ^ ((uint64_t)(p0 + cc) * 0xBF58476D1CE4E5B9ull);
            h ^= h >> 31; h *= 0x94D049BB133111EBull; h ^= h >> 29;
            v = (h & 1) ? 1.f : -1.f;
        } else v = (r == p0 + cc) ? 1.f : 0.f;
        Z[i] = v;
    }
}

}

using namespace gemb;

extern "C" int gemb_hope_svd_error(gemb_graph *g, int d, float beta, const float *X, int n_probe, uint64_t seed,
                                   double *err_out) {
    GEMB_ARG(g && X && err_out, "graph/X/err_out");
    GEMB_ARG(d >= 2 && d % 2 == 0, "d must be even");
    gemb_ctx *c = g->ctx;
    GEMB_ARG(c->nranks == 1 && g->n_local == g->n, "gemb_hope_svd_error is single-GPU");
    GEMB_CUDA(cudaSetDevice(c->device));
    const int64_t n = g->n;
    const int k = d / 2;
    const bool probe = n_probe > 0;
    const int w = (int)std::min<int64_t>(64, probe ? ((n_probe + 3) / 4 * 4) : ((n + 3) / 4 * 4));
    HopeWork W;
    W.g = g; W.c = c; W.b = w; W.rows = n; W.shard = n;
    const size_t blk = sizeof(float) * (size_t)n * w;
    for (int i = 0; i < 5; i++) { GEMB_CUDA(dmalloc(&W.buf[i], blk)); GEMB_CUDA(cudaMemsetAsync(W.buf[i], 0, blk, c->stream)); }
    GEMB_CUDA(dmalloc(&W.scal, sizeof(double) * (w + 8)));
    GEMB_CUDA(dmalloc(&W.G, sizeof(double) * (size_t)k * w));
    GEMB_CUDA(dmalloc(&W.M1, sizeof(float) * (size_t)k * w));
    float *Xd = nullptr, *L = nullptr, *Rr = nullptr;
    GEMB_CUDA(dmalloc(&Xd, sizeof(float) * (size_t)n * d));
    GEMB_CUDA(dmalloc(&L, sizeof(float) * (size_t)n * k));
    GEMB_CUDA(dmalloc(&Rr, sizeof(float) * (size_t)n * k));
    struct Guard { float *a, *b, *c; ~Guard() { dfree(a); dfree(b); dfree(c); } } guard{Xd, L, Rr};
    GEMB_CUDA(cudaMemcpyAsync(Xd, X, sizeof(float) * (size_t)n * d, cudaMemcpyHostToDevice, c->stream));
    split_halves_kernel<<<c->sm_count * 4, 256, 0, c->stream>>>(n, d, Xd, L, Rr);
    GEMB_CUDA(cudaGetLastError());
    count_launch();
    c->t_spmm.reset(); c->t_dense.reset(); c->t_comm.reset();
    double nrm = 0.0;
    GEMB_TRY(estimate_norm2(W, seed ? seed : 1, W.buf[3], W.buf[4], W.buf[2], &nrm));
    if ((double)beta * nrm * 1.02 >= 1.0) {
        set_error("beta * ||A||_2 = %.4g >= 1: the Katz series does not converge", (double)beta * nrm);
        return GEMB_ERR_DIVERGE;
    }
    const int J = katz_terms_for(beta, nrm, 1e-9);
    for (int i = 2; i < 5; i++) GEMB_CUDA(cudaMemsetAsync(W.buf[i], 0, blk, c->stream));
    float *Z = W.buf[0], *SZ = W.buf[1], *LZ = W.buf[2];
    const int64_t total_cols = probe ? n_probe : n;
    double acc = 0.0;
    std::vector<double> rs(w);
    const int threads = (256 / w) * w > 0 ? (256 / w) * w : w;
    for (int64_t p0 = 0; p0 < total_cols; p0 += w) {
        const int live = (int)std::min<int64_t>(w, total_cols - p0);
        probe_block_kernel<<<c->sm_count * 4, 256, 0, c->stream>>>(n, w, p0, probe ? 1 : 0, seed, Z);
        GEMB_CUDA(cudaGetLastError());
        count_launch();
        GEMB_TRY(katz(W, false, beta, J, Z, SZ, W.buf[3], W.buf[4]));
        GEMB_TRY(gram_launch(c, n, Rr, k, Z, w, W.G));
        f64_to_f32_kernel<<<(k * w + 255) / 256, 256, 0, c->stream>>>(k * w, W.G, W.M1);
        GEMB_CUDA(cudaGetLastError());
        count_launch();
        GEMB_TRY(apply_launch(c, n, L, k, W.M1, w, w, LZ, w));
        GEMB_CUDA(cudaMemsetAsync(W.scal, 0, sizeof(double) * w, c->stream));
        coldiff_sumsq_kernel<<<c->sm_count * 4, threads, 0, c->stream>>>(n, w, LZ, SZ, W.scal);
        GEMB_CUDA(cudaGetLastError());
        count_launch();
        GEMB_CUDA(cudaMemcpyAsync(rs.data(), W.scal, sizeof(double) * w, cudaMemcpyDeviceToHost, c->stream));
        GEMB_CUDA(cudaStreamSynchronize(c->stream));
        for (int j = 0; j < live; j++) acc += rs[j];
    }
    *err_out = sqrt(probe ? acc / (double)n_probe : acc);
    return GEMB_OK;
}

extern "C" int gemb_hope(gemb_graph *g, int d, float beta, const gemb_hope_opts *uo, float *X_out,
                         float *sigma_out, gemb_hope_stats *stats) {
    GEMB_ARG(g != nullptr, "graph");
    GEMB_ARG(d >= 1, "d must be >= 1");
    GEMB_ARG((uo && uo->struct_size == sizeof(gemb_hope_opts) && uo->spectral_mode == 1) || d % 2 == 0, "d must be even (k = d/2 singular triplets)");
    GEMB_ARG(!stats || stats->struct_size == sizeof(gemb_hope_stats), "stats.struct_size");
    gemb_ctx *c = g->ctx;
    GEMB_CUDA(cudaSetDevice(c->device));
    GEMB_ARG(!(c->nranks > 1 && g->replicated), "multi-GPU HOPE needs row shards (upload rows [rank*ceil(n/P), ...))");
    Opts o;
    if (uo) {
        GEMB_ARG(uo->struct_size == sizeof(gemb_hope_opts), "opts.struct_size");
        if (uo->oversample >= 0) o.oversample = uo->oversample;
        if (uo->max_iters > 0) o.max_iters = uo->max_iters;
        if (uo->min_iters > 0) o.min_iters = uo->min_iters;
        if (uo->tol > 0) o.tol = uo->tol;
        if (uo->katz_terms > 0) o.katz_terms = uo->katz_terms;
        if (uo->katz_tol > 0) o.katz_tol = uo->katz_tol;
        if (uo->seed) o.seed = uo->seed;
        o.compute_residual = uo->compute_residual;
        o.verbose = uo->verbose;
        GEMB_ARG(uo->algorithm >= 0 && uo->algorithm <= 3, "opts.algorithm");
        o.algorithm = uo->algorithm;
        if (uo->cheb_degree >= 2) o.cheb_degree = uo->cheb_degree;
        if (uo->cheb_range_log2 > 0.f) o.range_log2 = uo->cheb_range_log2;
        GEMB_ARG(uo->stop_rule == 0 || uo->stop_rule == 1, "opts.stop_rule");
        o.stop_rule = uo->stop_rule;
        if (uo->algorithm3_basis > 0) o.lanczos_basis = uo->algorithm3_basis;
        GEMB_ARG(uo->spectral_mode == 0 || uo->spectral_mode == 1, "opts.spectral_mode");
        o.spectral_mode = uo->spectral_mode;
    }
    if (o.spectral_mode == 1) {
        GEMB_ARG(g->symmetric, "spectral_mode 1 (largest algebraic eigenpairs) needs a symmetric upload");
        GEMB_ARG(o.algorithm == 0 || o.algorithm == 2, "spectral_mode 1 runs on the Chebyshev-filtered subspace iteration (algorithm 0 or 2)");
        o.algorithm = 2;
        beta = 0.f;
    }
    if (o.algorithm >= 2 && !g->symmetric) {
        set_error("algorithm=%d (works on A itself, S = f(A)) needs a symmetric shard (upload with indptr_t = NULL)", o.algorithm);
        return GEMB_ERR_ARG;
    }
    const int algo = o.algorithm ? o.algorithm : (g->symmetric ? 2 : 1);
    const int k = o.spectral_mode ? d : d / 2;
    GEMB_ARG((int64_t)k <= g->n, "d/2 must not exceed the number of nodes");
    int64_t bb = std::min<int64_t>(g->n, (int64_t)k + o.oversample);
    int b = (int)((bb + 3) / 4 * 4);
    GEMB_ARG(b <= 1024, "block width d/2 + oversample must be <= 1024");

    static const bool trace = getenv("GEMB_TRACE") != nullptr;
    auto now = [] { return std::chrono::duration<double, std::milli>(std::chrono::steady_clock::now().time_since_epoch()).count(); };
    const double t_enter = now();
    HopeWork W;
    W.g = g; W.c = c; W.b = b; W.rows = g->n_local; W.shard = g->n_shard;
    const size_t blk = sizeof(float) * (size_t)W.shard * b;
    static const bool mg_allgather = getenv("GEMB_MG") && !strcmp(getenv("GEMB_MG"), "allgather");
    if (c->nranks > 1 && algo >= 2 && !mg_allgather) {
        int hs = halo_build(g);
        if (hs == GEMB_OK) hs = halo_buffers(g, 5, b);
        NcclApi *api = nccl_api();
        if (!api) return GEMB_ERR_NCCL;
        int *flag = nullptr, hflag = (hs == GEMB_OK) ? 1 : 0;
        GEMB_CUDA(dmalloc(&flag, sizeof(int)));
        GEMB_CUDA(cudaMemcpyAsync(flag, &hflag, sizeof(int), cudaMemcpyHostToDevice, c->stream));
        ncclResult_t r = api->AllReduce(flag, flag, 1, ncclInt, ncclMin, (ncclComm_t)c->comm, c->stream);
        GEMB_CUDA(cudaMemcpyAsync(&hflag, flag, sizeof(int), cudaMemcpyDeviceToHost, c->stream));
        GEMB_CUDA(cudaStreamSynchronize(c->stream));
        dfree(flag);
        if (r != ncclSuccess) { set_error("ncclAllReduce(halo agreement): %s", api->GetErrorString(r)); return GEMB_ERR_NCCL; }
        W.halo = hflag == 1;
        if (W.halo) {
            const char *we = getenv("GEMB_WIRE");
            W.wire_half = we && !strcmp(we, "fp16-experimental");
        }
        if (!W.halo && o.verbose) fprintf(stderr, "[gemb_hope] halo exchange unavailable (%s); all-gather per sweep\n", gemb_last_error());
    }
    if (W.halo) {
        for (int i = 0; i < 5; i++) W.buf[i] = g->halo.buf[i];
        GEMB_TRY(halo_barrier(g));
    } else {
        for (int i = 0; i < 5; i++) {
            GEMB_CUDA(dmalloc(&W.buf[i], blk ? blk : 4));
            GEMB_CUDA(cudaMemsetAsync(W.buf[i], 0, blk, c->stream));
        }
        if (c->nranks > 1) GEMB_CUDA(dmalloc(&W.full, sizeof(float) * (size_t)g->n_pad * b));
    }
    GEMB_CUDA(dmalloc(&W.G, sizeof(double) * b * b));
    GEMB_CUDA(dmalloc(&W.G2, sizeof(double) * b * b));
    GEMB_CUDA(dmalloc(&W.Z, sizeof(double) * b * b));
    GEMB_CUDA(dmalloc(&W.Zs, sizeof(double) * b * b));
    GEMB_CUDA(dmalloc(&W.w, sizeof(double) * b));
    GEMB_CUDA(dmalloc(&W.scal, sizeof(double) * (b + 8)));
    GEMB_CUDA(dmalloc(&W.Minv, sizeof(float) * b * b));
    GEMB_CUDA(dmalloc(&W.M1, sizeof(float) * b * b));
    GEMB_CUDA(dmalloc(&W.M2, sizeof(float) * b * b));
    GEMB_CUDA(dmalloc(&W.rank_dev, sizeof(int)));

    c->t_spmm.reset(); c->t_dense.reset(); c->t_comm.reset(); c->t_misc.reset();
    const double t_alloc = now();
    cudaEvent_t ev0, ev1;
    GEMB_CUDA(cudaEventCreate(&ev0));
    GEMB_CUDA(cudaEventCreate(&ev1));
    GEMB_CUDA(cudaEventRecord(ev0, c->stream));

    double nrm = 0.0, hard_bound = 0.0;
    int J = o.katz_terms;
    bool have_nrm = false;
    if (beta < 0.f) {
        GEMB_TRY(estimate_norm2(W, o.seed, W.buf[3], W.buf[4], W.buf[2], &nrm));
        if (!(nrm > 0.0)) { set_error("beta < 0 asks for beta = |beta| / ||A||_2, but ||A||_2 = 0 (empty graph)"); cudaEventDestroy(ev0); cudaEventDestroy(ev1); return GEMB_ERR_ARG; }
        beta = (float)(-(double)beta / nrm);
        have_nrm = true;
        for (int i = 2; i < 5; i++) GEMB_CUDA(cudaMemsetAsync(W.buf[i], 0, blk, c->stream));
    }
    bool need_power = (J <= 0 && algo == 1) && !have_nrm;
    if (algo >= 2) {
        bool nonneg = false;
        GEMB_TRY(rowsum_bound(W, &hard_bound, &nonneg));
        if (nonneg && (double)beta * hard_bound * 1.02 < 1.0) nrm = -1.0;
        else need_power = !have_nrm;
    }
    if (have_nrm && nrm >= 0.0) {
        if ((double)beta * nrm * 1.02 >= 1.0) { set_error("|beta| / ||A||_2 with |beta| >= 0.98: outside the Katz convergence radius"); cudaEventDestroy(ev0); cudaEventDestroy(ev1); return GEMB_ERR_DIVERGE; }
        if (J <= 0) J = katz_terms_for(beta, nrm, o.katz_tol);
        if (hard_bound <= 0.0) hard_bound = nrm;
    }
    if (need_power) {
        GEMB_TRY(estimate_norm2(W, o.seed, W.buf[3], W.buf[4], W.buf[2], &nrm));
        if ((double)beta * nrm * 1.02 >= 1.0) {
            int Jp = 0;
            double rho = nrm;
            int ps = GEMB_ERR_DIVERGE;
            if (algo == 1 && !W.halo) {
                ps = probe_katz_terms(W, beta, o.katz_tol, o.seed, W.buf[3], W.buf[4], &Jp, &rho);
                if (ps != GEMB_OK && ps != GEMB_ERR_DIVERGE) { cudaEventDestroy(ev0); cudaEventDestroy(ev1); return ps; }
            }
            if (ps != GEMB_OK) {
                set_error("beta * rho(A) ~ %.4g >= 1 (||A||_2 = %.4g): the Katz series (I - beta A)^-1 beta A does not "
                          "converge; choose beta < %.4g", (double)beta * rho, nrm, 1.0 / std::max(rho, 1e-300));
                cudaEventDestroy(ev0); cudaEventDestroy(ev1);
                return GEMB_ERR_DIVERGE;
            }
            if (J <= 0) J = Jp;
        }
        if (J <= 0) J = katz_terms_for(beta, nrm, o.katz_tol);
        if (hard_bound <= 0.0) hard_bound = nrm;
        for (int i = 2; i < 5; i++) GEMB_CUDA(cudaMemsetAsync(W.buf[i], 0, blk, c->stream));
    }

    HopeResult R;
    int s;
    const bool lanczos_fits = g->n >= 2048;
    if (algo == 3 && lanczos_fits) s = hope_lanczos(W, o, d, beta, hard_bound > 0 ? hard_bound : nrm, R);
    else if (algo >= 2) {
        s = hope_symmetric(W, o, d, beta, nrm, hard_bound, R);
        if (s == GEMB_SWITCH_TO_LANCZOS) { R = HopeResult(); s = hope_lanczos(W, o, d, beta, hard_bound > 0 ? hard_bound : nrm, R); }
    } else s = hope_general(W, o, d, beta, J, R);
    if (s != GEMB_OK) { dfree(R.Xalloc); cudaEventDestroy(ev0); cudaEventDestroy(ev1); return s; }

    GEMB_CUDA(cudaEventRecord(ev1, c->stream));
    GEMB_CUDA(cudaEventSynchronize(ev1));
    if (W.halo) { const int hs = halo_check_timeout(g); if (hs != GEMB_OK) { dfree(R.Xalloc); cudaEventDestroy(ev0); cudaEventDestroy(ev1); return hs; } }
    float total_ms = 0.f;
    GEMB_CUDA(cudaEventElapsedTime(&total_ms, ev0, ev1));

    const double t_solve = now();
    double d2h_ms = 0.0;
    if (X_out || sigma_out) {
        cudaEvent_t e2, e3;
        GEMB_CUDA(cudaEventCreate(&e2)); GEMB_CUDA(cudaEventCreate(&e3));
        GEMB_CUDA(cudaEventRecord(e2, c->stream));
        if (X_out) GEMB_CUDA(cudaMemcpyAsync(X_out, R.Xd, sizeof(float) * (size_t)W.rows * d, cudaMemcpyDeviceToHost, c->stream));
        if (sigma_out) GEMB_CUDA(cudaMemcpyAsync(sigma_out, R.sig_dev, sizeof(float) * k, cudaMemcpyDeviceToHost, c->stream));
        GEMB_CUDA(cudaEventRecord(e3, c->stream));
        GEMB_CUDA(cudaEventSynchronize(e3));
        float ms = 0.f; cudaEventElapsedTime(&ms, e2, e3); d2h_ms = ms;
        cudaEventDestroy(e2); cudaEventDestroy(e3);
    }
    dfree(R.Xalloc);
    cudaEventDestroy(ev0); cudaEventDestroy(ev1);
    if (trace)
        fprintf(stderr, "[gemb_hope] host ms: alloc %.2f  solve %.2f (device %.2f)  d2h %.2f (device %.2f)\n",
                t_alloc - t_enter, t_solve - t_alloc, total_ms, now() - t_solve, d2h_ms);

    if (stats) {
        stats->iters = R.iters;
        stats->katz_terms = R.katz_terms;
        stats->block = b;
        stats->converged = R.converged;
        stats->algorithm = R.algorithm;
        stats->spmm_count = W.spmm_wide;
        stats->spmm_ms = c->t_spmm.total_ms();
        const double nnz = (double)g->A.nnz;
        double x_rows = (double)g->n;
        if (c->nranks > 1) x_rows = (double)W.rows + (W.halo ? (double)g->halo.halo_rows : 0.0);
        stats->spmm_bytes = (g->A.data ? 8.0 : 4.0) * nnz + 4.0 * (double)(W.rows + 1) +
                            4.0 * (double)b * (x_rows + (double)W.rows);
        stats->halo_rows = W.halo ? g->halo.halo_rows : 0;
        stats->push_rows = W.halo ? g->halo.push_total : 0;
        stats->pushes = W.pushes;
        stats->mg_mode = c->nranks == 1 ? 0 : (W.halo ? (W.wire_half ? 3 : 2) : 1);
        stats->push_bytes = W.halo ? W.push_bytes_per_row * (double)g->halo.push_total : 0.0;
        stats->resid_est = R.resid_est;
        stats->dense_ms = c->t_dense.total_ms();
        stats->comm_ms = c->t_comm.total_ms();
        stats->total_ms = total_ms;
        stats->h2d_ms = 0.0;
        stats->d2h_ms = d2h_ms;
        stats->norm2_A = (float)(nrm >= 0.0 ? nrm : hard_bound);
        stats->beta_used = beta;
        stats->ritz_change = (float)R.change;
        stats->resid_max = R.resid_max;
    }
    return GEMB_OK;
}
```

### gem_b200/csrc/tc_common.cuh

```cuda
#pragma once
#include "common.cuh"

namespace gemb {
namespace tc {

__device__ __forceinline__ uint32_t smem_u32(const void *p) { return (uint32_t)__cvta_generic_to_shared(p); }

__device__ __forceinline__ void mbar_init(uint32_t bar, uint32_t count) {
    asm volatile("mbarrier.init.shared::cta.b64 [%0], %1;" ::"r"(bar), "r"(count));
}
__device__ __forceinline__ bool mbar_try_wait(uint32_t bar, uint32_t parity) {
    uint32_t ok;
    asm volatile(
        "{\n.reg .pred p;\nmbarrier.try_wait.parity.shared::cta.b64 p, [%1], %2;\nselp.b32 %0, 1, 0, p;\n}"
        : "=r"(ok)
        : "r"(bar), "r"(parity)
        : "memory");
    return ok != 0;
}
__device__ __forceinline__ void mbar_wait(uint32_t bar, uint32_t parity) {
    for (uint32_t it = 0; it < (1u << 22); it++) {
        if (mbar_try_wait(bar, parity)) return;
        __nanosleep(40);
    }
    __trap();
}
__device__ __forceinline__ void mbar_arrive(uint32_t bar) {
    asm volatile("mbarrier.arrive.shared::cta.b64 _, [%0];" ::"r"(bar) : "memory");
}
__device__ __forceinline__ void mbar_expect_tx(uint32_t bar, uint32_t bytes) {
    asm volatile("mbarrier.arrive.expect_tx.shared::cta.b64 _, [%0], %1;" ::"r"(bar), "r"(bytes) : "memory");
}
__device__ __forceinline__ void bulk_g2s(uint32_t dst_smem, const void *src, uint32_t bytes, uint32_t bar) {
    asm volatile("cp.async.bulk.shared::cluster.global.mbarrier::complete_tx::bytes [%0], [%1], %2, [%3];"
                 ::"r"(dst_smem), "l"(src), "r"(bytes), "r"(bar) : "memory");
}
__device__ __forceinline__ void fence_proxy_async() { asm volatile("fence.proxy.async.shared::cta;" ::: "memory"); }
__device__ __forceinline__ void named_sync(uint32_t id, uint32_t count) {
    asm volatile("bar.sync %0, %1;" ::"r"(id), "r"(count) : "memory");
}

__device__ __forceinline__ uint32_t to_tf32(float x) {
    uint32_t r;
    asm("cvt.rna.tf32.f32 %0, %1;" : "=r"(r) : "f"(x));
    return r;
}
__device__ __forceinline__ void split_tf32(const float4 &v, uint4 &hi, uint4 &lo) {
    hi.x = to_tf32(v.x); hi.y = to_tf32(v.y); hi.z = to_tf32(v.z); hi.w = to_tf32(v.w);
    lo.x = to_tf32(v.x - __uint_as_float(hi.x));
    lo.y = to_tf32(v.y - __uint_as_float(hi.y));
    lo.z = to_tf32(v.z - __uint_as_float(hi.z));
    lo.w = to_tf32(v.w - __uint_as_float(hi.w));
}

__device__ __forceinline__ uint64_t make_desc(uint32_t smem_addr, uint32_t lbo_bytes, uint32_t sbo_bytes) {
    uint64_t d = 0;
    d |= (uint64_t)((smem_addr >> 4) & 0x3FFF);
    d |= (uint64_t)((lbo_bytes >> 4) & 0x3FFF) << 16;
    d |= (uint64_t)((sbo_bytes >> 4) & 0x3FFF) << 32;
    return d;
}

__device__ __forceinline__ void wgmma_fence() { asm volatile("wgmma.fence.sync.aligned;" ::: "memory"); }
__device__ __forceinline__ void wgmma_commit() { asm volatile("wgmma.commit_group.sync.aligned;" ::: "memory"); }
__device__ __forceinline__ void wgmma_wait_all() { asm volatile("wgmma.wait_group.sync.aligned 0;" ::: "memory"); }

template <int N> __device__ __forceinline__ void wgmma_tf32(float (&d)[N / 2], uint64_t a, uint64_t b, uint32_t scale_d);
template <> __device__ __forceinline__ void wgmma_tf32<32>(float (&d)[16], uint64_t a, uint64_t b, uint32_t scale_d) {
    asm volatile(
        "{\n.reg .pred p;\nsetp.ne.b32 p, %18, 0;\n"
        "wgmma.mma_async.sync.aligned.m64n32k8.f32.tf32.tf32 {"
        "%0, %1, %2, %3, %4, %5, %6, %7, %8, %9, %10, %11, %12, %13, %14, %15"
        "}, %16, %17, p, 1, 1;\n}\n"
        : "+f"(d[0]), "+f"(d[1]), "+f"(d[2]), "+f"(d[3]), "+f"(d[4]), "+f"(d[5]), "+f"(d[6]), "+f"(d[7]),
          "+f"(d[8]), "+f"(d[9]), "+f"(d[10]), "+f"(d[11]), "+f"(d[12]), "+f"(d[13]), "+f"(d[14]), "+f"(d[15])
        : "l"(a), "l"(b), "r"(scale_d));
}
template <> __device__ __forceinline__ void wgmma_tf32<64>(float (&d)[32], uint64_t a, uint64_t b, uint32_t scale_d) {
    asm volatile(
        "{\n.reg .pred p;\nsetp.ne.b32 p, %34, 0;\n"
        "wgmma.mma_async.sync.aligned.m64n64k8.f32.tf32.tf32 {"
        "%0, %1, %2, %3, %4, %5, %6, %7, %8, %9, %10, %11, %12, %13, %14, %15, "
        "%16, %17, %18, %19, %20, %21, %22, %23, %24, %25, %26, %27, %28, %29, %30, %31"
        "}, %32, %33, p, 1, 1;\n}\n"
        : "+f"(d[0]), "+f"(d[1]), "+f"(d[2]), "+f"(d[3]), "+f"(d[4]), "+f"(d[5]), "+f"(d[6]), "+f"(d[7]),
          "+f"(d[8]), "+f"(d[9]), "+f"(d[10]), "+f"(d[11]), "+f"(d[12]), "+f"(d[13]), "+f"(d[14]), "+f"(d[15]),
          "+f"(d[16]), "+f"(d[17]), "+f"(d[18]), "+f"(d[19]), "+f"(d[20]), "+f"(d[21]), "+f"(d[22]), "+f"(d[23]),
          "+f"(d[24]), "+f"(d[25]), "+f"(d[26]), "+f"(d[27]), "+f"(d[28]), "+f"(d[29]), "+f"(d[30]), "+f"(d[31])
        : "l"(a), "l"(b), "r"(scale_d));
}
template <> __device__ __forceinline__ void wgmma_tf32<80>(float (&d)[40], uint64_t a, uint64_t b, uint32_t scale_d) {
    asm volatile(
        "{\n.reg .pred p;\nsetp.ne.b32 p, %42, 0;\n"
        "wgmma.mma_async.sync.aligned.m64n80k8.f32.tf32.tf32 {"
        "%0, %1, %2, %3, %4, %5, %6, %7, %8, %9, %10, %11, %12, %13, %14, %15, "
        "%16, %17, %18, %19, %20, %21, %22, %23, %24, %25, %26, %27, %28, %29, %30, %31, "
        "%32, %33, %34, %35, %36, %37, %38, %39"
        "}, %40, %41, p, 1, 1;\n}\n"
        : "+f"(d[0]), "+f"(d[1]), "+f"(d[2]), "+f"(d[3]), "+f"(d[4]), "+f"(d[5]), "+f"(d[6]), "+f"(d[7]),
          "+f"(d[8]), "+f"(d[9]), "+f"(d[10]), "+f"(d[11]), "+f"(d[12]), "+f"(d[13]), "+f"(d[14]), "+f"(d[15]),
          "+f"(d[16]), "+f"(d[17]), "+f"(d[18]), "+f"(d[19]), "+f"(d[20]), "+f"(d[21]), "+f"(d[22]), "+f"(d[23]),
          "+f"(d[24]), "+f"(d[25]), "+f"(d[26]), "+f"(d[27]), "+f"(d[28]), "+f"(d[29]), "+f"(d[30]), "+f"(d[31]),
          "+f"(d[32]), "+f"(d[33]), "+f"(d[34]), "+f"(d[35]), "+f"(d[36]), "+f"(d[37]), "+f"(d[38]), "+f"(d[39])
        : "l"(a), "l"(b), "r"(scale_d));
}
template <> __device__ __forceinline__ void wgmma_tf32<96>(float (&d)[48], uint64_t a, uint64_t b, uint32_t scale_d) {
    asm volatile(
        "{\n.reg .pred p;\nsetp.ne.b32 p, %50, 0;\n"
        "wgmma.mma_async.sync.aligned.m64n96k8.f32.tf32.tf32 {"
        "%0, %1, %2, %3, %4, %5, %6, %7, %8, %9, %10, %11, %12, %13, %14, %15, "
        "%16, %17, %18, %19, %20, %21, %22, %23, %24, %25, %26, %27, %28, %29, %30, %31, "
        "%32, %33, %34, %35, %36, %37, %38, %39, %40, %41, %42, %43, %44, %45, %46, %47"
        "}, %48, %49, p, 1, 1;\n}\n"
        : "+f"(d[0]), "+f"(d[1]), "+f"(d[2]), "+f"(d[3]), "+f"(d[4]), "+f"(d[5]), "+f"(d[6]), "+f"(d[7]),
          "+f"(d[8]), "+f"(d[9]), "+f"(d[10]), "+f"(d[11]), "+f"(d[12]), "+f"(d[13]), "+f"(d[14]), "+f"(d[15]),
          "+f"(d[16]), "+f"(d[17]), "+f"(d[18]), "+f"(d[19]), "+f"(d[20]), "+f"(d[21]), "+f"(d[22]), "+f"(d[23]),
          "+f"(d[24]), "+f"(d[25]), "+f"(d[26]), "+f"(d[27]), "+f"(d[28]), "+f"(d[29]), "+f"(d[30]), "+f"(d[31]),
          "+f"(d[32]), "+f"(d[33]), "+f"(d[34]), "+f"(d[35]), "+f"(d[36]), "+f"(d[37]), "+f"(d[38]), "+f"(d[39]),
          "+f"(d[40]), "+f"(d[41]), "+f"(d[42]), "+f"(d[43]), "+f"(d[44]), "+f"(d[45]), "+f"(d[46]), "+f"(d[47])
        : "l"(a), "l"(b), "r"(scale_d));
}
template <> __device__ __forceinline__ void wgmma_tf32<128>(float (&d)[64], uint64_t a, uint64_t b, uint32_t scale_d) {
    asm volatile(
        "{\n.reg .pred p;\nsetp.ne.b32 p, %66, 0;\n"
        "wgmma.mma_async.sync.aligned.m64n128k8.f32.tf32.tf32 {"
        "%0, %1, %2, %3, %4, %5, %6, %7, %8, %9, %10, %11, %12, %13, %14, %15, "
        "%16, %17, %18, %19, %20, %21, %22, %23, %24, %25, %26, %27, %28, %29, %30, %31, "
        "%32, %33, %34, %35, %36, %37, %38, %39, %40, %41, %42, %43, %44, %45, %46, %47, "
        "%48, %49, %50, %51, %52, %53, %54, %55, %56, %57, %58, %59, %60, %61, %62, %63"
        "}, %64, %65, p, 1, 1;\n}\n"
        : "+f"(d[0]), "+f"(d[1]), "+f"(d[2]), "+f"(d[3]), "+f"(d[4]), "+f"(d[5]), "+f"(d[6]), "+f"(d[7]),
          "+f"(d[8]), "+f"(d[9]), "+f"(d[10]), "+f"(d[11]), "+f"(d[12]), "+f"(d[13]), "+f"(d[14]), "+f"(d[15]),
          "+f"(d[16]), "+f"(d[17]), "+f"(d[18]), "+f"(d[19]), "+f"(d[20]), "+f"(d[21]), "+f"(d[22]), "+f"(d[23]),
          "+f"(d[24]), "+f"(d[25]), "+f"(d[26]), "+f"(d[27]), "+f"(d[28]), "+f"(d[29]), "+f"(d[30]), "+f"(d[31]),
          "+f"(d[32]), "+f"(d[33]), "+f"(d[34]), "+f"(d[35]), "+f"(d[36]), "+f"(d[37]), "+f"(d[38]), "+f"(d[39]),
          "+f"(d[40]), "+f"(d[41]), "+f"(d[42]), "+f"(d[43]), "+f"(d[44]), "+f"(d[45]), "+f"(d[46]), "+f"(d[47]),
          "+f"(d[48]), "+f"(d[49]), "+f"(d[50]), "+f"(d[51]), "+f"(d[52]), "+f"(d[53]), "+f"(d[54]), "+f"(d[55]),
          "+f"(d[56]), "+f"(d[57]), "+f"(d[58]), "+f"(d[59]), "+f"(d[60]), "+f"(d[61]), "+f"(d[62]), "+f"(d[63])
        : "l"(a), "l"(b), "r"(scale_d));
}

}
}
```

Baseline: 14.91 million.

## Tighten WGMMA widths, pipeline gram stages, move Ritz quad to GPU, fuse applies

Tensor-core kernels now use N widths padded only to the next multiple of 8, so less padded work is done. The gram kernel double-buffers accumulators to overlap consecutive stages, and adds a narrow-slice path for the second warpgroup when the row count is between 64 and 120. The Ritz residual quadratic form is now computed on the GPU instead of copying two b×b matrices to the host and looping there. The two apply launches are fused into one with concatenated coefficient matrices. The cost is many more template instantiations and a more complex gram code path.

New measurement: 15.11 million, median of 6. +1.3%, better.

```diff
diff --git a/gem_b200/csrc/apply_tc.cu b/gem_b200/csrc/apply_tc.cu
--- a/gem_b200/csrc/apply_tc.cu
+++ b/gem_b200/csrc/apply_tc.cu
@@ -145,20 +145,17 @@
 
 template <int TILE_M>
 static int apply_tc_dispatch(gemb_ctx *ctx, const ApplyTcParams &p, int npad, int grid, size_t smem_bytes) {
-    switch (npad) {
-        case 32: return apply_tc_launch_t<TILE_M, 32>(ctx, p, grid, smem_bytes);
-        case 64: return apply_tc_launch_t<TILE_M, 64>(ctx, p, grid, smem_bytes);
-        case 80: return apply_tc_launch_t<TILE_M, 80>(ctx, p, grid, smem_bytes);
-        case 96: return apply_tc_launch_t<TILE_M, 96>(ctx, p, grid, smem_bytes);
+    switch (npad / 8) {
+#define GEMB_APPLY_CASE(g) case g: return apply_tc_launch_t<TILE_M, 8 * g>(ctx, p, grid, smem_bytes);
+        GEMB_APPLY_CASE(1) GEMB_APPLY_CASE(2) GEMB_APPLY_CASE(3) GEMB_APPLY_CASE(4) GEMB_APPLY_CASE(5) GEMB_APPLY_CASE(6)
+        GEMB_APPLY_CASE(7) GEMB_APPLY_CASE(8) GEMB_APPLY_CASE(9) GEMB_APPLY_CASE(10) GEMB_APPLY_CASE(11) GEMB_APPLY_CASE(12)
+        GEMB_APPLY_CASE(13) GEMB_APPLY_CASE(14) GEMB_APPLY_CASE(15)
+#undef GEMB_APPLY_CASE
         default: return apply_tc_launch_t<TILE_M, 128>(ctx, p, grid, smem_bytes);
     }
 }
 
-static int pad_width(int b) {
-    const int widths[5] = {32, 64, 80, 96, 128};
-    for (int w : widths) if (w >= b) return w;
-    return 128;
-}
+static int pad_width(int b) { return (b + 7) / 8 * 8; }
 
 static size_t apply_smem_bytes(int tile_m, int b1, int npad) {
     const size_t raw_slot = (size_t)tile_m * b1 * 4, a_tile = (size_t)(b1 / 4) * (16 * tile_m + 16);
diff --git a/gem_b200/csrc/gram_tc.cu b/gem_b200/csrc/gram_tc.cu
--- a/gem_b200/csrc/gram_tc.cu
+++ b/gem_b200/csrc/gram_tc.cu
@@ -104,21 +104,24 @@
         }
     } else {
         const int wg = warp >> 2;
-        const bool active = wg * 64 < p.mb;
-        float acc[NPAD / 2], racc[NPAD / 2];
-#pragma unroll
-        for (int i = 0; i < NPAD / 2; i++) racc[i] = 0.f;
-        for (int it = 0; it < nst; it++) {
-            const int st = it & 1;
-            tc::mbar_wait(tc::smem_u32(&s_tile_full[st]), (uint32_t)(it >> 1) & 1);
-            if (active) {
-                const uint32_t a_hi = tc::smem_u32(tile_base + (size_t)st * stage_bytes), a_lo = a_hi + p.tile_bytes_a;
-                const uint32_t b_hi = BSEP ? a_hi + 2 * p.tile_bytes_a : a_hi;
-                const uint32_t b_lo = BSEP ? b_hi + p.tile_bytes_b : a_lo;
-                const uint32_t a_off = (uint32_t)wg * 8u * sbo;
+        const uint32_t step = (uint32_t)((2u * lbo) >> 4);
+        auto tiles = [&](int st, uint32_t &a_hi, uint32_t &a_lo, uint32_t &b_hi, uint32_t &b_lo) {
+            a_hi = tc::smem_u32(tile_base + (size_t)st * stage_bytes); a_lo = a_hi + p.tile_bytes_a;
+            b_hi = BSEP ? a_hi + 2 * p.tile_bytes_a : a_hi;
+            b_lo = BSEP ? b_hi + p.tile_bytes_b : a_lo;
+        };
+        const bool rem = p.mb > 64 && p.mb <= 120;
+        if (wg == 0 || !rem) {
+            const bool active = wg * 64 < p.mb;
+            const uint32_t a_off = (uint32_t)wg * 8u * sbo;
+            float acc0[NPAD / 2], acc1[NPAD / 2], racc[NPAD / 2];
+#pragma unroll
+            for (int i = 0; i < NPAD / 2; i++) racc[i] = 0.f;
+            auto issue = [&](float (&acc)[NPAD / 2], int it) {
+                uint32_t a_hi, a_lo, b_hi, b_lo;
+                tiles(it & 1, a_hi, a_lo, b_hi, b_lo);
                 uint64_t dah = tc::make_desc(a_hi + a_off, lbo, sbo), dal = tc::make_desc(a_lo + a_off, lbo, sbo);
                 uint64_t dbh = tc::make_desc(b_hi, lbo, sbo), dbl = tc::make_desc(b_lo, lbo, sbo);
-                const uint64_t step = (uint64_t)((2u * lbo) >> 4);
                 tc::wgmma_fence();
                 for (int kb = 0; kb < kblocks; kb++) {
                     tc::wgmma_tf32<NPAD>(acc, dah, dbh, kb > 0 ? 1u : 0u);
@@ -127,22 +130,109 @@
                     dah += step; dal += step; dbh += step; dbl += step;
                 }
                 tc::wgmma_commit();
+            };
+            auto fold = [&](float (&acc)[NPAD / 2]) {
+#pragma unroll
+                for (int i = 0; i < NPAD / 2; i++) racc[i] += acc[i];
+            };
+            auto release = [&](int it) { __syncwarp(); if (lane == 0) tc::mbar_arrive(tc::smem_u32(&s_tile_free[it & 1])); };
+            if (!active) {
+                for (int it = 0; it < nst; it++) {
+                    tc::mbar_wait(tc::smem_u32(&s_tile_full[it & 1]), (uint32_t)(it >> 1) & 1);
+                    release(it);
+                }
+            } else if (NPAD <= 80) {
+                auto stage = [&](float (&cur)[NPAD / 2], float (&prev)[NPAD / 2], int it) {
+                    tc::mbar_wait(tc::smem_u32(&s_tile_full[it & 1]), (uint32_t)(it >> 1) & 1);
+                    issue(cur, it);
+                    if (it > 0) { tc::wgmma_wait_1(); release(it - 1); fold(prev); }
+                };
+                for (int it = 0; it < nst; it++) {
+                    if (it & 1) stage(acc1, acc0, it);
+                    else stage(acc0, acc1, it);
+                }
                 tc::wgmma_wait_all();
-            }
-            __syncwarp();
-            if (lane == 0) tc::mbar_arrive(tc::smem_u32(&s_tile_free[st]));
+                if (nst > 0) { release(nst - 1); if ((nst - 1) & 1) fold(acc1); else fold(acc0); }
+            } else {
+                for (int it = 0; it < nst; it++) {
+                    tc::mbar_wait(tc::smem_u32(&s_tile_full[it & 1]), (uint32_t)(it >> 1) & 1);
+                    issue(acc0, it);
+                    tc::wgmma_wait_all();
+                    release(it);
+                    fold(acc0);
+                }
+            }
             if (active) {
-#pragma unroll
-                for (int i = 0; i < NPAD / 2; i++) racc[i] += acc[i];
-            }
-        }
-        if (active) {
-            const int r0 = wg * 64 + (warp & 3) * 16 + (lane >> 2);
+                const int r0 = wg * 64 + (warp & 3) * 16 + (lane >> 2);
+                double *dst = p.part + (size_t)blockIdx.x * p.part_stride + (size_t)p.m0 * p.ldg + p.n0;
+#pragma unroll
+                for (int i = 0; i < NPAD / 2; i++) {
+                    const int row = r0 + ((i >> 1) & 1) * 8, col = (i >> 2) * 8 + (lane & 3) * 2 + (i & 1);
+                    if (row < p.mb && col < p.nb) dst[(size_t)row * p.ldg + col] = (double)racc[i];
+                }
+            }
+        } else {
+            const int nslices = (p.mb - 64 + 7) / 8;
+            const int nb8 = (p.nb + 7) / 8 * 8;
+            const int last = nb8 > 64 ? nb8 - 64 : 0;
+            const int nchunks = last == 0 ? 1 : 2;
+            float acc[2][7][4], racc[2][7][4];
+#pragma unroll
+            for (int c = 0; c < 2; c++)
+#pragma unroll
+                for (int s = 0; s < 7; s++)
+#pragma unroll
+                    for (int i = 0; i < 4; i++) racc[c][s][i] = acc[c][s][i] = 0.f;
+            for (int it = 0; it < nst; it++) {
+                tc::mbar_wait(tc::smem_u32(&s_tile_full[it & 1]), (uint32_t)(it >> 1) & 1);
+                uint32_t a_hi, a_lo, b_hi, b_lo;
+                tiles(it & 1, a_hi, a_lo, b_hi, b_lo);
+                tc::wgmma_fence();
+#pragma unroll
+                for (int c = 0; c < 2; c++) {
+                    if (c >= nchunks) break;
+                    const uint32_t c_off = (uint32_t)(c == 0 ? 0 : last / 8) * sbo;
+#pragma unroll
+                    for (int s = 0; s < 7; s++) {
+                        if (s >= nslices) break;
+                        const uint32_t s_off = (uint32_t)(8 + s) * sbo;
+                        uint64_t dmh = tc::make_desc(b_hi + c_off, lbo, sbo), dml = tc::make_desc(b_lo + c_off, lbo, sbo);
+                        uint64_t dnh = tc::make_desc(a_hi + s_off, lbo, sbo), dnl = tc::make_desc(a_lo + s_off, lbo, sbo);
+                        for (int kb = 0; kb < kblocks; kb++) {
+                            tc::wgmma_tf32<8>(acc[c][s], dmh, dnh, kb > 0 ? 1u : 0u);
+                            tc::wgmma_tf32<8>(acc[c][s], dml, dnh, 1u);
+                            tc::wgmma_tf32<8>(acc[c][s], dmh, dnl, 1u);
+                            dmh += step; dml += step; dnh += step; dnl += step;
+                        }
+                    }
+                }
+                tc::wgmma_commit();
+                tc::wgmma_wait_all();
+                __syncwarp();
+                if (lane == 0) tc::mbar_arrive(tc::smem_u32(&s_tile_free[it & 1]));
+#pragma unroll
+                for (int c = 0; c < 2; c++)
+#pragma unroll
+                    for (int s = 0; s < 7; s++)
+#pragma unroll
+                        for (int i = 0; i < 4; i++) racc[c][s][i] += acc[c][s][i];
+            }
             double *dst = p.part + (size_t)blockIdx.x * p.part_stride + (size_t)p.m0 * p.ldg + p.n0;
 #pragma unroll
-            for (int i = 0; i < NPAD / 2; i++) {
-                const int row = r0 + ((i >> 1) & 1) * 8, col = (i >> 2) * 8 + (lane & 3) * 2 + (i & 1);
-                if (row < p.mb && col < p.nb) dst[(size_t)row * p.ldg + col] = (double)racc[i];
+            for (int c = 0; c < 2; c++) {
+                if (c >= nchunks) break;
+                const int c0 = c == 0 ? 0 : last;
+                const int cmin = c == 0 ? 0 : 64;
+#pragma unroll
+                for (int s = 0; s < 7; s++) {
+                    if (s >= nslices) break;
+#pragma unroll
+                    for (int i = 0; i < 4; i++) {
+                        const int row = 64 + 8 * s + (lane & 3) * 2 + (i & 1);
+                        const int col = c0 + (warp & 3) * 16 + (lane >> 2) + (i >> 1) * 8;
+                        if (row < p.mb && col >= cmin && col < p.nb) dst[(size_t)row * p.ldg + col] = (double)racc[c][s][i];
+                    }
+                }
             }
         }
     }
@@ -163,11 +253,14 @@
 
 template <bool QRAW, bool BSEP>
 static int gram_tc_dispatch(gemb_ctx *ctx, const GramTcParams &p, int grid, size_t smem_bytes) {
-    if (p.nb <= 32) return gram_tc_launch_t<QRAW, BSEP, 32>(ctx, p, grid, smem_bytes);
-    if (p.nb <= 64) return gram_tc_launch_t<QRAW, BSEP, 64>(ctx, p, grid, smem_bytes);
-    if (p.nb <= 80) return gram_tc_launch_t<QRAW, BSEP, 80>(ctx, p, grid, smem_bytes);
-    if (p.nb <= 96) return gram_tc_launch_t<QRAW, BSEP, 96>(ctx, p, grid, smem_bytes);
-    return gram_tc_launch_t<QRAW, BSEP, 128>(ctx, p, grid, smem_bytes);
+    switch ((p.nb + 7) / 8) {
+#define GEMB_GRAM_CASE(g) case g: return gram_tc_launch_t<QRAW, BSEP, 8 * g>(ctx, p, grid, smem_bytes);
+        GEMB_GRAM_CASE(1) GEMB_GRAM_CASE(2) GEMB_GRAM_CASE(3) GEMB_GRAM_CASE(4) GEMB_GRAM_CASE(5) GEMB_GRAM_CASE(6)
+        GEMB_GRAM_CASE(7) GEMB_GRAM_CASE(8) GEMB_GRAM_CASE(9) GEMB_GRAM_CASE(10) GEMB_GRAM_CASE(11) GEMB_GRAM_CASE(12)
+        GEMB_GRAM_CASE(13) GEMB_GRAM_CASE(14) GEMB_GRAM_CASE(15)
+#undef GEMB_GRAM_CASE
+        default: return gram_tc_launch_t<QRAW, BSEP, 128>(ctx, p, grid, smem_bytes);
+    }
 }
 
 int gram_tc_launch(gemb_ctx *ctx, int64_t n, const float *P, int b1, const float *Q, int b2, double *G) {
diff --git a/gem_b200/csrc/hope.cu b/gem_b200/csrc/hope.cu
--- a/gem_b200/csrc/hope.cu
+++ b/gem_b200/csrc/hope.cu
@@ -194,6 +194,23 @@
         acc += d * d;
     }
     atomicAdd(out + j, acc);
+}
+
+__global__ void __launch_bounds__(128) ritz_quad_kernel(int b, const double *__restrict__ G, const double *__restrict__ Z,
+                                                        double *__restrict__ q) {
+    extern __shared__ double s_t[];
+    const int j = blockIdx.x;
+    for (int r = threadIdx.x; r < b; r += blockDim.x) {
+        double t = 0.0;
+        for (int c = 0; c < b; c++) t = __dadd_rn(t, __dmul_rn(G[(size_t)r * b + c], Z[(size_t)c * b + j]));
+        s_t[r] = t;
+    }
+    __syncthreads();
+    if (threadIdx.x == 0) {
+        double acc = 0.0;
+        for (int r = 0; r < b; r++) acc = __dadd_rn(acc, __dmul_rn(Z[(size_t)r * b + j], s_t[r]));
+        q[j] = acc;
+    }
 }
 
 __global__ void symmetrize_kernel(int b, double *__restrict__ T) {
@@ -578,8 +595,7 @@
         }
     }
 
-    std::vector<double> lam(b), gval(b), th_sorted(b), th_prev(b, 0.0);
-    std::vector<double> Wh(o.stop_rule == 1 ? (size_t)b * b : 0), Zr(o.stop_rule == 1 ? (size_t)b * b : 0);
+    std::vector<double> lam(2 * b), gval(b), th_sorted(b), th_prev(b, 0.0);
     std::vector<int> order(b);
     struct Plan { bool valid = false; int deg = 0; double e = 0, c0 = 0, sigma1 = 0; } plan;
 
@@ -615,7 +631,13 @@
         GEMB_TRY(c->t_dense.begin(c->stream));
         GEMB_TRY(eigh_launch(c, b, W.G2, W.w, W.Z, W.Zs, std::min(1e-5, std::max(1e-13, 1e-2 * (double)o.tol))));
         GEMB_TRY(c->t_dense.end(c->stream));
-        GEMB_CUDA(cudaMemcpyAsync(lam.data(), W.w, sizeof(double) * b, cudaMemcpyDeviceToHost, c->stream));
+        if (o.stop_rule == 1) {
+            GEMB_TRY(gram_full(W, AV, AV, W.G));
+            ritz_quad_kernel<<<b, 128, sizeof(double) * b, c->stream>>>(b, W.G, W.Z, W.w + b);
+            GEMB_CUDA(cudaGetLastError());
+            count_launch();
+        }
+        GEMB_CUDA(cudaMemcpyAsync(lam.data(), W.w, sizeof(double) * (o.stop_rule == 1 ? 2 * b : b), cudaMemcpyDeviceToHost, c->stream));
         GEMB_CUDA(cudaStreamSynchronize(c->stream));
         float *filtered = nullptr;
         if (ritz_bound) {
@@ -643,19 +665,10 @@
             return GEMB_SWITCH_TO_LANCZOS;
         double stop_measure = change;
         if (o.stop_rule == 1) {
-            GEMB_TRY(gram_full(W, AV, AV, W.G));
-            GEMB_CUDA(cudaMemcpyAsync(Wh.data(), W.G, sizeof(double) * b * b, cudaMemcpyDeviceToHost, c->stream));
-            GEMB_CUDA(cudaMemcpyAsync(Zr.data(), W.Z, sizeof(double) * b * b, cudaMemcpyDeviceToHost, c->stream));
-            GEMB_CUDA(cudaStreamSynchronize(c->stream));
             double worst = 0.0;
             for (int j = 0; j < k; j++) {
                 const int col = order[j];
-                double q = 0.0;
-                for (int r = 0; r < b; r++) {
-                    double t = 0.0;
-                    for (int s2 = 0; s2 < b; s2++) t += Wh[(size_t)r * b + s2] * Zr[(size_t)s2 * b + col];
-                    q += Zr[(size_t)r * b + col] * t;
-                }
+                const double q = lam[b + col];
                 const double l = std::max(-bound, std::min(bound, lam[col]));
                 const double r2 = std::max(q - lam[col] * lam[col], 0.0);
                 const double fp = mode ? 1.0 : (double)beta / ((1.0 - beta * l) * (1.0 - beta * l));
@@ -733,7 +746,7 @@
     std::vector<double> Zh((size_t)b * b);
     GEMB_CUDA(cudaMemcpyAsync(Zh.data(), W.Z, sizeof(double) * b * b, cudaMemcpyDeviceToHost, c->stream));
     GEMB_CUDA(cudaStreamSynchronize(c->stream));
-    std::vector<float> M1((size_t)b * k), M2((size_t)b * k), sig(k);
+    std::vector<float> M12((size_t)b * 2 * k), sig(k);
     for (int j = 0; j < k; j++) {
         const int col = sel[j];
         const double l = std::max(-bound, std::min(bound, lam[col]));
@@ -741,13 +754,12 @@
         sig[j] = (float)sg;
         for (int i = 0; i < b; i++) {
             const double z = Zh[(size_t)i * b + col];
-            M2[(size_t)i * k + j] = (float)(z * rt);
-            M1[(size_t)i * k + j] = (float)((f < 0 ? -z : z) * rt);
+            M12[(size_t)i * 2 * k + k + j] = (float)(z * rt);
+            M12[(size_t)i * 2 * k + j] = (float)((f < 0 ? -z : z) * rt);
         }
     }
     R.sigma_max = gval[order[0]];
-    GEMB_CUDA(cudaMemcpyAsync(W.M1, M1.data(), sizeof(float) * b * k, cudaMemcpyHostToDevice, c->stream));
-    GEMB_CUDA(cudaMemcpyAsync(W.M2, M2.data(), sizeof(float) * b * k, cudaMemcpyHostToDevice, c->stream));
+    GEMB_CUDA(cudaMemcpyAsync(W.M1, M12.data(), sizeof(float) * b * 2 * k, cudaMemcpyHostToDevice, c->stream));
     R.sig_dev = (float *)W.G2;
     GEMB_CUDA(cudaMemcpyAsync(R.sig_dev, sig.data(), sizeof(float) * k, cudaMemcpyHostToDevice, c->stream));
     GEMB_CUDA(cudaStreamSynchronize(c->stream));
@@ -757,8 +769,7 @@
         R.Xd = R.Xalloc;
     }
     GEMB_TRY(c->t_dense.begin(c->stream));
-    GEMB_TRY(apply_launch(c, W.rows, V, b, W.M1, k, k, R.Xd, d));
-    GEMB_TRY(apply_launch(c, W.rows, V, b, W.M2, k, k, R.Xd + k, d));
+    GEMB_TRY(apply_launch(c, W.rows, V, b, W.M1, 2 * k, 2 * k, R.Xd, d));
     GEMB_TRY(c->t_dense.end(c->stream));
 
     if (o.compute_residual) {
@@ -1229,10 +1240,10 @@
     GEMB_CUDA(dmalloc(&W.G2, sizeof(double) * b * b));
     GEMB_CUDA(dmalloc(&W.Z, sizeof(double) * b * b));
     GEMB_CUDA(dmalloc(&W.Zs, sizeof(double) * b * b));
-    GEMB_CUDA(dmalloc(&W.w, sizeof(double) * b));
+    GEMB_CUDA(dmalloc(&W.w, sizeof(double) * 2 * b));
     GEMB_CUDA(dmalloc(&W.scal, sizeof(double) * (b + 8)));
     GEMB_CUDA(dmalloc(&W.Minv, sizeof(float) * b * b));
-    GEMB_CUDA(dmalloc(&W.M1, sizeof(float) * b * b));
+    GEMB_CUDA(dmalloc(&W.M1, sizeof(float) * 2 * b * b));
     GEMB_CUDA(dmalloc(&W.M2, sizeof(float) * b * b));
     GEMB_CUDA(dmalloc(&W.rank_dev, sizeof(int)));
 
diff --git a/gem_b200/csrc/tc_common.cuh b/gem_b200/csrc/tc_common.cuh
--- a/gem_b200/csrc/tc_common.cuh
+++ b/gem_b200/csrc/tc_common.cuh
@@ -64,81 +64,187 @@
 __device__ __forceinline__ void wgmma_fence() { asm volatile("wgmma.fence.sync.aligned;" ::: "memory"); }
 __device__ __forceinline__ void wgmma_commit() { asm volatile("wgmma.commit_group.sync.aligned;" ::: "memory"); }
 __device__ __forceinline__ void wgmma_wait_all() { asm volatile("wgmma.wait_group.sync.aligned 0;" ::: "memory"); }
+__device__ __forceinline__ void wgmma_wait_1() { asm volatile("wgmma.wait_group.sync.aligned 1;" ::: "memory"); }
 
 template <int N> __device__ __forceinline__ void wgmma_tf32(float (&d)[N / 2], uint64_t a, uint64_t b, uint32_t scale_d);
+#define GEMB_D4(i) "+f"(d[i]), "+f"(d[i + 1]), "+f"(d[i + 2]), "+f"(d[i + 3])
+template <> __device__ __forceinline__ void wgmma_tf32<8>(float (&d)[4], uint64_t a, uint64_t b, uint32_t scale_d) {
+    asm volatile("{\n.reg .pred p;\nsetp.ne.b32 p, %6, 0;\n"
+                 "wgmma.mma_async.sync.aligned.m64n8k8.f32.tf32.tf32 {"
+                 "%0, %1, %2, %3"
+                 "}, %4, %5, p, 1, 1;\n}\n"
+                 : GEMB_D4(0)
+                 : "l"(a), "l"(b), "r"(scale_d));
+}
+template <> __device__ __forceinline__ void wgmma_tf32<16>(float (&d)[8], uint64_t a, uint64_t b, uint32_t scale_d) {
+    asm volatile("{\n.reg .pred p;\nsetp.ne.b32 p, %10, 0;\n"
+                 "wgmma.mma_async.sync.aligned.m64n16k8.f32.tf32.tf32 {"
+                 "%0, %1, %2, %3, %4, %5, %6, %7"
+                 "}, %8, %9, p, 1, 1;\n}\n"
+                 : GEMB_D4(0), GEMB_D4(4)
+                 : "l"(a), "l"(b), "r"(scale_d));
+}
+template <> __device__ __forceinline__ void wgmma_tf32<24>(float (&d)[12], uint64_t a, uint64_t b, uint32_t scale_d) {
+    asm volatile("{\n.reg .pred p;\nsetp.ne.b32 p, %14, 0;\n"
+                 "wgmma.mma_async.sync.aligned.m64n24k8.f32.tf32.tf32 {"
+                 "%0, %1, %2, %3, %4, %5, %6, %7, %8, %9, %10, %11"
+                 "}, %12, %13, p, 1, 1;\n}\n"
+                 : GEMB_D4(0), GEMB_D4(4), GEMB_D4(8)
+                 : "l"(a), "l"(b), "r"(scale_d));
+}
 template <> __device__ __forceinline__ void wgmma_tf32<32>(float (&d)[16], uint64_t a, uint64_t b, uint32_t scale_d) {
-    asm volatile(
-        "{\n.reg .pred p;\nsetp.ne.b32 p, %18, 0;\n"
-        "wgmma.mma_async.sync.aligned.m64n32k8.f32.tf32.tf32 {"
-        "%0, %1, %2, %3, %4, %5, %6, %7, %8, %9, %10, %11, %12, %13, %14, %15"
-        "}, %16, %17, p, 1, 1;\n}\n"
-        : "+f"(d[0]), "+f"(d[1]), "+f"(d[2]), "+f"(d[3]), "+f"(d[4]), "+f"(d[5]), "+f"(d[6]), "+f"(d[7]),
-          "+f"(d[8]), "+f"(d[9]), "+f"(d[10]), "+f"(d[11]), "+f"(d[12]), "+f"(d[13]), "+f"(d[14]), "+f"(d[15])
-        : "l"(a), "l"(b), "r"(scale_d));
+    asm volatile("{\n.reg .pred p;\nsetp.ne.b32 p, %18, 0;\n"
+                 "wgmma.mma_async.sync.aligned.m64n32k8.f32.tf32.tf32 {"
+                 "%0, %1, %2, %3, %4, %5, %6, %7, %8, %9, %10, %11, %12, %13, %14, %15"
+                 "}, %16, %17, p, 1, 1;\n}\n"
+                 : GEMB_D4(0), GEMB_D4(4), GEMB_D4(8), GEMB_D4(12)
+                 : "l"(a), "l"(b), "r"(scale_d));
+}
+template <> __device__ __forceinline__ void wgmma_tf32<40>(float (&d)[20], uint64_t a, uint64_t b, uint32_t scale_d) {
+    asm volatile("{\n.reg .pred p;\nsetp.ne.b32 p, %22, 0;\n"
+                 "wgmma.mma_async.sync.aligned.m64n40k8.f32.tf32.tf32 {"
+                 "%0, %1, %2, %3, %4, %5, %6, %7, %8, %9, %10, %11, %12, %13, %14, %15, "
+                 "%16, %17, %18, %19"
+                 "}, %20, %21, p, 1, 1;\n}\n"
+                 : GEMB_D4(0), GEMB_D4(4), GEMB_D4(8), GEMB_D4(12),
+                   GEMB_D4(16)
+                 : "l"(a), "l"(b), "r"(scale_d));
+}
+template <> __device__ __forceinline__ void wgmma_tf32<48>(float (&d)[24], uint64_t a, uint64_t b, uint32_t scale_d) {
+    asm volatile("{\n.reg .pred p;\nsetp.ne.b32 p, %26, 0;\n"
+                 "wgmma.mma_async.sync.aligned.m64n48k8.f32.tf32.tf32 {"
+                 "%0, %1, %2, %3, %4, %5, %6, %7, %8, %9, %10, %11, %12, %13, %14, %15, "
+                 "%16, %17, %18, %19, %20, %21, %22, %23"
+                 "}, %24, %25, p, 1, 1;\n}\n"
+                 : GEMB_D4(0), GEMB_D4(4), GEMB_D4(8), GEMB_D4(12),
+                   GEMB_D4(16), GEMB_D4(20)
+                 : "l"(a), "l"(b), "r"(scale_d));
+}
+template <> __device__ __forceinline__ void wgmma_tf32<56>(float (&d)[28], uint64_t a, uint64_t b, uint32_t scale_d) {
+    asm volatile("{\n.reg .pred p;\nsetp.ne.b32 p, %30, 0;\n"
+                 "wgmma.mma_async.sync.aligned.m64n56k8.f32.tf32.tf32 {"
+                 "%0, %1, %2, %3, %4, %5, %6, %7, %8, %9, %10, %11, %12, %13, %14, %15, "
+                 "%16, %17, %18, %19, %20, %21, %22, %23, %24, %25, %26, %27"
+                 "}, %28, %29, p, 1, 1;\n}\n"
+                 : GEMB_D4(0), GEMB_D4(4), GEMB_D4(8), GEMB_D4(12),
+                   GEMB_D4(16), GEMB_D4(20), GEMB_D4(24)
+                 : "l"(a), "l"(b), "r"(scale_d));
 }
 template <> __device__ __forceinline__ void wgmma_tf32<64>(float (&d)[32], uint64_t a, uint64_t b, uint32_t scale_d) {
-    asm volatile(
-        "{\n.reg .pred p;\nsetp.ne.b32 p, %34, 0;\n"
-        "wgmma.mma_async.sync.aligned.m64n64k8.f32.tf32.tf32 {"
-        "%0, %1, %2, %3, %4, %5, %6, %7, %8, %9, %10, %11, %12, %13, %14, %15, "
-        "%16, %17, %18, %19, %20, %21, %22, %23, %24, %25, %26, %27, %28, %29, %30, %31"
-        "}, %32, %33, p, 1, 1;\n}\n"
-        : "+f"(d[0]), "+f"(d[1]), "+f"(d[2]), "+f"(d[3]), "+f"(d[4]), "+f"(d[5]), "+f"(d[6]), "+f"(d[7]),
-          "+f"(d[8]), "+f"(d[9]), "+f"(d[10]), "+f"(d[11]), "+f"(d[12]), "+f"(d[13]), "+f"(d[14]), "+f"(d[15]),
-          "+f"(d[16]), "+f"(d[17]), "+f"(d[18]), "+f"(d[19]), "+f"(d[20]), "+f"(d[21]), "+f"(d[22]), "+f"(d[23]),
-          "+f"(d[24]), "+f"(d[25]), "+f"(d[26]), "+f"(d[27]), "+f"(d[28]), "+f"(d[29]), "+f"(d[30]), "+f"(d[31])
-        : "l"(a), "l"(b), "r"(scale_d));
+    asm volatile("{\n.reg .pred p;\nsetp.ne.b32 p, %34, 0;\n"
+                 "wgmma.mma_async.sync.aligned.m64n64k8.f32.tf32.tf32 {"
+                 "%0, %1, %2, %3, %4, %5, %6, %7, %8, %9, %10, %11, %12, %13, %14, %15, "
+                 "%16, %17, %18, %19, %20, %21, %22, %23, %24, %25, %26, %27, %28, %29, %30, %31"
+                 "}, %32, %33, p, 1, 1;\n}\n"
+                 : GEMB_D4(0), GEMB_D4(4), GEMB_D4(8), GEMB_D4(12),
+                   GEMB_D4(16), GEMB_D4(20), GEMB_D4(24), GEMB_D4(28)
+                 : "l"(a), "l"(b), "r"(scale_d));
+}
+template <> __device__ __forceinline__ void wgmma_tf32<72>(float (&d)[36], uint64_t a, uint64_t b, uint32_t scale_d) {
+    asm volatile("{\n.reg .pred p;\nsetp.ne.b32 p, %38, 0;\n"
+                 "wgmma.mma_async.sync.aligned.m64n72k8.f32.tf32.tf32 {"
+                 "%0, %1, %2, %3, %4, %5, %6, %7, %8, %9, %10, %11, %12, %13, %14, %15, "
+                 "%16, %17, %18, %19, %20, %21, %22, %23, %24, %25, %26, %27, %28, %29, %30, %31, "
+                 "%32, %33, %34, %35"
+                 "}, %36, %37, p, 1, 1;\n}\n"
+                 : GEMB_D4(0), GEMB_D4(4), GEMB_D4(8), GEMB_D4(12),
+                   GEMB_D4(16), GEMB_D4(20), GEMB_D4(24), GEMB_D4(28),
+                   GEMB_D4(32)
+                 : "l"(a), "l"(b), "r"(scale_d));
 }
 template <> __device__ __forceinline__ void wgmma_tf32<80>(float (&d)[40], uint64_t a, uint64_t b, uint32_t scale_d) {
-    asm volatile(
-        "{\n.reg .pred p;\nsetp.ne.b32 p, %42, 0;\n"
-        "wgmma.mma_async.sync.aligned.m64n80k8.f32.tf32.tf32 {"
-        "%0, %1, %2, %3, %4, %5, %6, %7, %8, %9, %10, %11, %12, %13, %14, %15, "
-        "%16, %17, %18, %19, %20, %21, %22, %23, %24, %25, %26, %27, %28, %29, %30, %31, "
-        "%32, %33, %34, %35, %36, %37, %38, %39"
-        "}, %40, %41, p, 1, 1;\n}\n"
-        : "+f"(d[0]), "+f"(d[1]), "+f"(d[2]), "+f"(d[3]), "+f"(d[4]), "+f"(d[5]), "+f"(d[6]), "+f"(d[7]),
-          "+f"(d[8]), "+f"(d[9]), "+f"(d[10]), "+f"(d[11]), "+f"(d[12]), "+f"(d[13]), "+f"(d[14]), "+f"(d[15]),
-          "+f"(d[16]), "+f"(d[17]), "+f"(d[18]), "+f"(d[19]), "+f"(d[20]), "+f"(d[21]), "+f"(d[22]), "+f"(d[23]),
-          "+f"(d[24]), "+f"(d[25]), "+f"(d[26]), "+f"(d[27]), "+f"(d[28]), "+f"(d[29]), "+f"(d[30]), "+f"(d[31]),
-          "+f"(d[32]), "+f"(d[33]), "+f"(d[34]), "+f"(d[35]), "+f"(d[36]), "+f"(d[37]), "+f"(d[38]), "+f"(d[39])
-        : "l"(a), "l"(b), "r"(scale_d));
+    asm volatile("{\n.reg .pred p;\nsetp.ne.b32 p, %42, 0;\n"
+                 "wgmma.mma_async.sync.aligned.m64n80k8.f32.tf32.tf32 {"
+                 "%0, %1, %2, %3, %4, %5, %6, %7, %8, %9, %10, %11, %12, %13, %14, %15, "
+                 "%16, %17, %18, %19, %20, %21, %22, %23, %24, %25, %26, %27, %28, %29, %30, %31, "
+                 "%32, %33, %34, %35, %36, %37, %38, %39"
+                 "}, %40, %41, p, 1, 1;\n}\n"
+                 : GEMB_D4(0), GEMB_D4(4), GEMB_D4(8), GEMB_D4(12),
+                   GEMB_D4(16), GEMB_D4(20), GEMB_D4(24), GEMB_D4(28),
+                   GEMB_D4(32), GEMB_D4(36)
+                 : "l"(a), "l"(b), "r"(scale_d));
+}
+template <> __device__ __forceinline__ void wgmma_tf32<88>(float (&d)[44], uint64_t a, uint64_t b, uint32_t scale_d) {
+    asm volatile("{\n.reg .pred p;\nsetp.ne.b32 p, %46, 0;\n"
+                 "wgmma.mma_async.sync.aligned.m64n88k8.f32.tf32.tf32 {"
+                 "%0, %1, %2, %3, %4, %5, %6, %7, %8, %9, %10, %11, %12, %13, %14, %15, "
+                 "%16, %17, %18, %19, %20, %21, %22, %23, %24, %25, %26, %27, %28, %29, %30, %31, "
+                 "%32, %33, %34, %35, %36, %37, %38, %39, %40, %41, %42, %43"
+                 "}, %44, %45, p, 1, 1;\n}\n"
+                 : GEMB_D4(0), GEMB_D4(4), GEMB_D4(8), GEMB_D4(12),
+                   GEMB_D4(16), GEMB_D4(20), GEMB_D4(24), GEMB_D4(28),
+                   GEMB_D4(32), GEMB_D4(36), GEMB_D4(40)
+                 : "l"(a), "l"(b), "r"(scale_d));
 }
 template <> __device__ __forceinline__ void wgmma_tf32<96>(float (&d)[48], uint64_t a, uint64_t b, uint32_t scale_d) {
-    asm volatile(
-        "{\n.reg .pred p;\nsetp.ne.b32 p, %50, 0;\n"
-        "wgmma.mma_async.sync.aligned.m64n96k8.f32.tf32.tf32 {"
-        "%0, %1, %2, %3, %4, %5, %6, %7, %8, %9, %10, %11, %12, %13, %14, %15, "
-        "%16, %17, %18, %19, %20, %21, %22, %23, %24, %25, %26, %27, %28, %29, %30, %31, "
-        "%32, %33, %34, %35, %36, %37, %38, %39, %40, %41, %42, %43, %44, %45, %46, %47"
-        "}, %48, %49, p, 1, 1;\n}\n"
-        : "+f"(d[0]), "+f"(d[1]), "+f"(d[2]), "+f"(d[3]), "+f"(d[4]), "+f"(d[5]), "+f"(d[6]), "+f"(d[7]),
-          "+f"(d[8]), "+f"(d[9]), "+f"(d[10]), "+f"(d[11]), "+f"(d[12]), "+f"(d[13]), "+f"(d[14]), "+f"(d[15]),
-          "+f"(d[16]), "+f"(d[17]), "+f"(d[18]), "+f"(d[19]), "+f"(d[20]), "+f"(d[21]), "+f"(d[22]), "+f"(d[23]),
-          "+f"(d[24]), "+f"(d[25]), "+f"(d[26]), "+f"(d[27]), "+f"(d[28]), "+f"(d[29]), "+f"(d[30]), "+f"(d[31]),
-          "+f"(d[32]), "+f"(d[33]), "+f"(d[34]), "+f"(d[35]), "+f"(d[36]), "+f"(d[37]), "+f"(d[38]), "+f"(d[39]),
-          "+f"(d[40]), "+f"(d[41]), "+f"(d[42]), "+f"(d[43]), "+f"(d[44]), "+f"(d[45]), "+f"(d[46]), "+f"(d[47])
-        : "l"(a), "l"(b), "r"(scale_d));
+    asm volatile("{\n.reg .pred p;\nsetp.ne.b32 p, %50, 0;\n"
+                 "wgmma.mma_async.sync.aligned.m64n96k8.f32.tf32.tf32 {"
+                 "%0, %1, %2, %3, %4, %5, %6, %7, %8, %9, %10, %11, %12, %13, %14, %15, "
+                 "%16, %17, %18, %19, %20, %21, %22, %23, %24, %25, %26, %27, %28, %29, %30, %31, "
+                 "%32, %33, %34, %35, %36, %37, %38, %39, %40, %41, %42, %43, %44, %45, %46, %47"
+                 "}, %48, %49, p, 1, 1;\n}\n"
+                 : GEMB_D4(0), GEMB_D4(4), GEMB_D4(8), GEMB_D4(12),
+                   GEMB_D4(16), GEMB_D4(20), GEMB_D4(24), GEMB_D4(28),
+                   GEMB_D4(32), GEMB_D4(36), GEMB_D4(40), GEMB_D4(44)
+                 : "l"(a), "l"(b), "r"(scale_d));
+}
+template <> __device__ __forceinline__ void wgmma_tf32<104>(float (&d)[52], uint64_t a, uint64_t b, uint32_t scale_d) {
+    asm volatile("{\n.reg .pred p;\nsetp.ne.b32 p, %54, 0;\n"
+                 "wgmma.mma_async.sync.aligned.m64n104k8.f32.tf32.tf32 {"
+                 "%0, %1, %2, %3, %4, %5, %6, %7, %8, %9, %10, %11, %12, %13, %14, %15, "
+                 "%16, %17, %18, %19, %20, %21, %22, %23, %24, %25, %26, %27, %28, %29, %30, %31, "
+                 "%32, %33, %34, %35, %36, %37, %38, %39, %40, %41, %42, %43, %44, %45, %46, %47, "
+                 "%48, %49, %50, %51"
+                 "}, %52, %53, p, 1, 1;\n}\n"
+                 : GEMB_D4(0), GEMB_D4(4), GEMB_D4(8), GEMB_D4(12),
+                   GEMB_D4(16), GEMB_D4(20), GEMB_D4(24), GEMB_D4(28),
+                   GEMB_D4(32), GEMB_D4(36), GEMB_D4(40), GEMB_D4(44),
+                   GEMB_D4(48)
+                 : "l"(a), "l"(b), "r"(scale_d));
+}
+template <> __device__ __forceinline__ void wgmma_tf32<112>(float (&d)[56], uint64_t a, uint64_t b, uint32_t scale_d) {
+    asm volatile("{\n.reg .pred p;\nsetp.ne.b32 p, %58, 0;\n"
+                 "wgmma.mma_async.sync.aligned.m64n112k8.f32.tf32.tf32 {"
+                 "%0, %1, %2, %3, %4, %5, %6, %7, %8, %9, %10, %11, %12, %13, %14, %15, "
+                 "%16, %17, %18, %19, %20, %21, %22, %23, %24, %25, %26, %27, %28, %29, %30, %31, "
+                 "%32, %33, %34, %35, %36, %37, %38, %39, %40, %41, %42, %43, %44, %45, %46, %47, "
+                 "%48, %49, %50, %51, %52, %53, %54, %55"
+                 "}, %56, %57, p, 1, 1;\n}\n"
+                 : GEMB_D4(0), GEMB_D4(4), GEMB_D4(8), GEMB_D4(12),
+                   GEMB_D4(16), GEMB_D4(20), GEMB_D4(24), GEMB_D4(28),
+                   GEMB_D4(32), GEMB_D4(36), GEMB_D4(40), GEMB_D4(44),
+                   GEMB_D4(48), GEMB_D4(52)
+                 : "l"(a), "l"(b), "r"(scale_d));
+}
+template <> __device__ __forceinline__ void wgmma_tf32<120>(float (&d)[60], uint64_t a, uint64_t b, uint32_t scale_d) {
+    asm volatile("{\n.reg .pred p;\nsetp.ne.b32 p, %62, 0;\n"
+                 "wgmma.mma_async.sync.aligned.m64n120k8.f32.tf32.tf32 {"
+                 "%0, %1, %2, %3, %4, %5, %6, %7, %8, %9, %10, %11, %12, %13, %14, %15, "
+                 "%16, %17, %18, %19, %20, %21, %22, %23, %24, %25, %26, %27, %28, %29, %30, %31, "
+                 "%32, %33, %34, %35, %36, %37, %38, %39, %40, %41, %42, %43, %44, %45, %46, %47, "
+                 "%48, %49, %50, %51, %52, %53, %54, %55, %56, %57, %58, %59"
+                 "}, %60, %61, p, 1, 1;\n}\n"
+                 : GEMB_D4(0), GEMB_D4(4), GEMB_D4(8), GEMB_D4(12),
+                   GEMB_D4(16), GEMB_D4(20), GEMB_D4(24), GEMB_D4(28),
+                   GEMB_D4(32), GEMB_D4(36), GEMB_D4(40), GEMB_D4(44),
+                   GEMB_D4(48), GEMB_D4(52), GEMB_D4(56)
+                 : "l"(a), "l"(b), "r"(scale_d));
 }
 template <> __device__ __forceinline__ void wgmma_tf32<128>(float (&d)[64], uint64_t a, uint64_t b, uint32_t scale_d) {
-    asm volatile(
-        "{\n.reg .pred p;\nsetp.ne.b32 p, %66, 0;\n"
-        "wgmma.mma_async.sync.aligned.m64n128k8.f32.tf32.tf32 {"
-        "%0, %1, %2, %3, %4, %5, %6, %7, %8, %9, %10, %11, %12, %13, %14, %15, "
-        "%16, %17, %18, %19, %20, %21, %22, %23, %24, %25, %26, %27, %28, %29, %30, %31, "
-        "%32, %33, %34, %35, %36, %37, %38, %39, %40, %41, %42, %43, %44, %45, %46, %47, "
-        "%48, %49, %50, %51, %52, %53, %54, %55, %56, %57, %58, %59, %60, %61, %62, %63"
-        "}, %64, %65, p, 1, 1;\n}\n"
-        : "+f"(d[0]), "+f"(d[1]), "+f"(d[2]), "+f"(d[3]), "+f"(d[4]), "+f"(d[5]), "+f"(d[6]), "+f"(d[7]),
-          "+f"(d[8]), "+f"(d[9]), "+f"(d[10]), "+f"(d[11]), "+f"(d[12]), "+f"(d[13]), "+f"(d[14]), "+f"(d[15]),
-          "+f"(d[16]), "+f"(d[17]), "+f"(d[18]), "+f"(d[19]), "+f"(d[20]), "+f"(d[21]), "+f"(d[22]), "+f"(d[23]),
-          "+f"(d[24]), "+f"(d[25]), "+f"(d[26]), "+f"(d[27]), "+f"(d[28]), "+f"(d[29]), "+f"(d[30]), "+f"(d[31]),
-          "+f"(d[32]), "+f"(d[33]), "+f"(d[34]), "+f"(d[35]), "+f"(d[36]), "+f"(d[37]), "+f"(d[38]), "+f"(d[39]),
-          "+f"(d[40]), "+f"(d[41]), "+f"(d[42]), "+f"(d[43]), "+f"(d[44]), "+f"(d[45]), "+f"(d[46]), "+f"(d[47]),
-          "+f"(d[48]), "+f"(d[49]), "+f"(d[50]), "+f"(d[51]), "+f"(d[52]), "+f"(d[53]), "+f"(d[54]), "+f"(d[55]),
-          "+f"(d[56]), "+f"(d[57]), "+f"(d[58]), "+f"(d[59]), "+f"(d[60]), "+f"(d[61]), "+f"(d[62]), "+f"(d[63])
-        : "l"(a), "l"(b), "r"(scale_d));
-}
-
-}
-}
+    asm volatile("{\n.reg .pred p;\nsetp.ne.b32 p, %66, 0;\n"
+                 "wgmma.mma_async.sync.aligned.m64n128k8.f32.tf32.tf32 {"
+                 "%0, %1, %2, %3, %4, %5, %6, %7, %8, %9, %10, %11, %12, %13, %14, %15, "
+                 "%16, %17, %18, %19, %20, %21, %22, %23, %24, %25, %26, %27, %28, %29, %30, %31, "
+                 "%32, %33, %34, %35, %36, %37, %38, %39, %40, %41, %42, %43, %44, %45, %46, %47, "
+                 "%48, %49, %50, %51, %52, %53, %54, %55, %56, %57, %58, %59, %60, %61, %62, %63"
+                 "}, %64, %65, p, 1, 1;\n}\n"
+                 : GEMB_D4(0), GEMB_D4(4), GEMB_D4(8), GEMB_D4(12),
+                   GEMB_D4(16), GEMB_D4(20), GEMB_D4(24), GEMB_D4(28),
+                   GEMB_D4(32), GEMB_D4(36), GEMB_D4(40), GEMB_D4(44),
+                   GEMB_D4(48), GEMB_D4(52), GEMB_D4(56), GEMB_D4(60)
+                 : "l"(a), "l"(b), "r"(scale_d));
+}
+#undef GEMB_D4
+
+}
+}
```
